# Simple-Robotics/LoIK

Measured on AMD Instinct MI355X. Metric: IK solves/sec to 1e-6 residual, Talos humanoid, batch=65536 per GPU, higher is better.
Workload: dtype f64

## Files before the change

### loik_amd/csrc/loik_device.hpp

```cpp
#pragma once

#include <hip/hip_runtime.h>

namespace loikb {

constexpr int WAVE = 64;

enum : int {
  JP_CS = 0,
  JP_V = 1,
  JP_F = 4,
  JP_G = 7,
  JP_WZ = 10,
  JP_NUS = 11,
  JP_P = 12,
  JP_R = 15,
  JP_LBUB = 16,
  JP_UD = 17,
  JREC = 20,
  JP_NPERSIST = 12,
  CP_Y = 0,
  CP_ATY = 3,
  CP_B = 6,
  CP_ATB = 9,
  CREC_SHARED_A = 12,
  CP_A = 12,
  CP_ATA = 30,
  CREC_FULL = 42,
  SP_MU = 0,
  SP_BI = 1,
  SP_ST = 2,
  SP_TAG = 3,
  SP_FLIP = 4,
  SP_SCAL = 5,
  SREC = 20,
};

struct Layout {
  int nb, nc;
  int crec;
  int off_c;
  int off_s;
  int tile_pairs;
};

enum : int {
  JF_PARENT_ROOT = 2,
  JF_MASSLESS = 4,
  JF_NOQ = 8,
  JF_REVOLUTE = 16,
  JF_CS_DIRECT = 32,
  JF_HELICAL = 64,
};

enum : int { ROT_X = 0, ROT_Y = 1, ROT_Z = 2, ROT_U = 3, ROT_NONE = 4, ROT_FREE = 5, ROT_SPH = 6, ROT_TRANS = 7, ROT_PLANAR = 8 };

struct JointDesc {
  double Rp[9];
  double tp[3];
  double axis[3];
  int parent;
  int flags;
  int cslot;
  int rot;
  double pitch;
};

enum : int { ST_CONVERGED = 1, ST_PRIMAL_INF = 2, ST_TAIL = 4, ST_DONE = 8,
             ST_PFULL = 16 };

enum : int {
  MODE_FIXED_ITERS = 1,
  MODE_CACHE_H = 2,
  MODE_A_SHARED = 4,
  MODE_BND_SHARED = 8,
  MODE_MU_OSQP = 16,
  MODE_ZERO_STATE = 32,
  MODE_FLAT_PREP = 64,
};


enum : int {
  SC_PRIMAL_RES = 0, SC_DUAL_RES, SC_PRIMAL_RES_TASK, SC_PRIMAL_RES_SLACK, SC_DUAL_RES_V, SC_DUAL_RES_NU,
  SC_TOL_PRIMAL, SC_TOL_DUAL, SC_MU, SC_MU_EQ, SC_MU_INEQ,
  SC_DELTA_X_QP, SC_DELTA_Z_QP, SC_DELTA_Y_QP, SC_AT_DELTA_Y_QP, SC_UB_DY_PLUS, SC_LB_DY_MINUS,
  SC_DELTA_FIS, SC_DELTA_YIS, SC_DELTA_W, SC_DELTA_VIS, SC_DELTA_NU,
  SC_AV_INF, SC_NU_INF, SC_HREF_V_INF, SC_G_INF, SC_STF_PLUS_W_INF,
  SC_COND1, SC_COND2, SC_TAIL_ITER,
  NSCAL
};
static_assert(SP_SCAL + (NSCAL + 1) / 2 <= SREC, "scalar record too small");

template <typename T>
struct Params {
  T Href[36];
  T Hv[6];
  T Hv_inf_norm;
  const T* href_tab;
  T rho, mu0, mu_scale;
  T tol_abs, tol_rel, tol_primal_inf, tol_tail_solve;
  int max_iter;
  int mode;
  int B;
  int max_launch_iters;
  Layout L;
};

template <typename T>
struct Bufs {
  char* tiles;
  const T* uni;
  unsigned int* counters;
  int* wave_live;
  double* log;
  int* log_rows;
  int log_cap, log_B;
};

template <typename T> struct Vec2;
template <> struct Vec2<double> { using type = double2; };
template <> struct Vec2<float> { using type = float2; };

template <typename T>
__host__ __device__ constexpr size_t pair_bytes() { return (size_t)WAVE * 2 * sizeof(T); }

template <typename T>
__device__ __forceinline__ typename Vec2<T>::type ldp(const char* rec, int p)
{
  return *reinterpret_cast<const typename Vec2<T>::type*>(rec + (size_t)p * pair_bytes<T>());
}
template <typename T>
__device__ __forceinline__ void stp(char* rec, int p, T x, T y)
{
  typename Vec2<T>::type v;
  v.x = x; v.y = y;
  *reinterpret_cast<typename Vec2<T>::type*>(rec + (size_t)p * pair_bytes<T>()) = v;
}
template <typename T>
__device__ __forceinline__ void st_lo(char* rec, int p, T x) { *reinterpret_cast<T*>(rec + (size_t)p * pair_bytes<T>()) = x; }
template <typename T>
__device__ __forceinline__ void st_hi(char* rec, int p, T x) { *reinterpret_cast<T*>(rec + (size_t)p * pair_bytes<T>() + sizeof(T)) = x; }

template <typename T>
__device__ __forceinline__ void ld6(const char* rec, int p, T* x)
{
#pragma unroll
  for (int k = 0; k < 3; ++k) {
    const typename Vec2<T>::type v = ldp<T>(rec, p + k);
    x[2 * k] = v.x; x[2 * k + 1] = v.y;
  }
}
template <typename T>
__device__ __forceinline__ void st6(char* rec, int p, const T* x)
{
#pragma unroll
  for (int k = 0; k < 3; ++k) stp<T>(rec, p + k, x[2 * k], x[2 * k + 1]);
}

__host__ __device__ constexpr int sym(int i, int j)
{
  return (i <= j) ? (i * 6 - (i * (i - 1)) / 2 + (j - i)) : (j * 6 - (j * (j - 1)) / 2 + (i - j));
}

__host__ __device__ __forceinline__ double tabs(double x) { return __builtin_fabs(x); }
__host__ __device__ __forceinline__ float tabs(float x) { return __builtin_fabsf(x); }
__host__ __device__ __forceinline__ double tmax(double a, double b) { return __builtin_fmax(a, b); }
__host__ __device__ __forceinline__ float tmax(float a, float b) { return __builtin_fmaxf(a, b); }
__host__ __device__ __forceinline__ double tmin(double a, double b) { return __builtin_fmin(a, b); }
__host__ __device__ __forceinline__ float tmin(float a, float b) { return __builtin_fminf(a, b); }

template <typename T>
__device__ __forceinline__ bool update_mu(int mode, T primal, T dual, T norm_p, T norm_d, T& mu, int& kexp)
{
  if (mode & MODE_MU_OSQP) {
    const T rp = primal / (norm_p + T(1e-10)), rd = dual / (norm_d + T(1e-10));
    T mu_new = mu * (T)__builtin_sqrt((double)(rp / (rd + T(1e-10))));
    mu_new = tmin(tmax(mu_new, T(1e-6)), T(1e6));
    if (mu_new > T(5.0) * mu || mu_new < T(0.2) * mu) { mu = mu_new; return true; }
    return false;
  }
  if (primal > T(10) * dual) { mu *= T(10); ++kexp; return true; }
  if (dual > T(10) * primal) { mu *= T(0.1); --kexp; return true; }
  return false;
}

template <typename T>
__device__ __forceinline__ T inf6(const T* x)
{
  T m = tabs(x[0]);
#pragma unroll
  for (int k = 1; k < 6; ++k) m = tmax(m, tabs(x[k]));
  return m;
}

template <typename T>
__device__ __forceinline__ void cross3(const T* a, const T* b, T* o)
{
  o[0] = a[1] * b[2] - a[2] * b[1];
  o[1] = a[2] * b[0] - a[0] * b[2];
  o[2] = a[0] * b[1] - a[1] * b[0];
}

template <typename T>
__device__ __forceinline__ void mat3_vec(const T* A, const T* x, T* y)
{
#pragma unroll
  for (int i = 0; i < 3; ++i) y[i] = A[3 * i] * x[0] + A[3 * i + 1] * x[1] + A[3 * i + 2] * x[2];
}

template <typename T>
__device__ __forceinline__ void mat3t_vec(const T* A, const T* x, T* y)
{
#pragma unroll
  for (int i = 0; i < 3; ++i) y[i] = A[i] * x[0] + A[3 + i] * x[1] + A[6 + i] * x[2];
}

template <typename T>
__device__ __forceinline__ void make_liMi(const JointDesc& d, T c, T s, T* R, T* t)
{
  T Rp[9], tp[3], ax[3];
#pragma unroll
  for (int k = 0; k < 9; ++k) Rp[k] = (T)d.Rp[k];
#pragma unroll
  for (int k = 0; k < 3; ++k) { tp[k] = (T)d.tp[k]; ax[k] = (T)d.axis[k]; }
  if (d.flags & JF_REVOLUTE) {
    if (d.rot == ROT_X) {
#pragma unroll
      for (int i = 0; i < 3; ++i) {
        R[3 * i] = Rp[3 * i];
        R[3 * i + 1] = Rp[3 * i + 1] * c + Rp[3 * i + 2] * s;
        R[3 * i + 2] = Rp[3 * i + 2] * c - Rp[3 * i + 1] * s;
// ... 1518 lines not shown
```

### loik_amd/csrc/loik_flat_prep.hpp

```cpp
#pragma once

#include "loik_lean.hpp"

namespace loikb {

enum : int { C2_LANE = 0, C2_B = 2, C2_Y = 8, C2_ATYW = 14 , C2_ATBW = 20,
             C2_ATYF = 26 , C2_CW = 32, C2_DLT = 38 ,
             C2_VC = 44 , C2_ATY = 50 , C2_AW = 56, C2_AWT = 92,
             C2_A = 128, C2D = 164 };

constexpr int PREP_G = 32;
enum : int { PR_RT = 0, PR_JS = PR_RT + 12 * PREP_G, PR_SW = PR_JS + 4 * PREP_G, PR_SC = PR_SW + 3 * WAVE, PR_C = PR_SC + 32 };
enum : int { PRS_BNORM = 0, PRS_TGIN = 1, PRS_STY = 2, PRS_MU = 11, PRS_KEXP, PRS_ITER, PRS_STATUS, PRS_TAILIT, PRS_FLIP, PRS_N };

__host__ __device__ __forceinline__ int flat_prep_stride(int nc) { return PR_C + nc * C2D; }

template <typename T>
__device__ __forceinline__ T prep_awy_of(const T* blk, int k)
{
  const T* r = blk + C2_AW + 6 * k;
  const T* y = blk + C2_Y;
  return ((r[0] * y[0] + r[1] * y[1]) + r[2] * y[2]) + ((r[3] * y[3] + r[4] * y[4]) + r[5] * y[5]);
}
template <typename T>
__device__ __forceinline__ T prep_aty_of(const T* blk, int k)
{
  const T* A_ = blk + C2_A + k;
  const T* y = blk + C2_Y;
  return ((A_[0] * y[0] + A_[6] * y[1]) + A_[12] * y[2]) + ((A_[18] * y[3] + A_[24] * y[4]) + A_[30] * y[5]);
}

constexpr int PREP_NC = 4;
static_assert((WAVE / PREP_G) * PREP_NC * C2D <= (WAVE + 1) * 22, "the constraint blocks are built in k_fslots' placement rows");

template <typename T>
struct FlatPrepIn {
  typename Vec2<T>::type nus, lu;
  T sc;
  T cv[PREP_NC];
  T ca[PREP_NC][2];
};
template <typename T>
__device__ __forceinline__ void flat_prep_fetch(FlatPrepIn<T>& in, bool has_inst, const Params<T>& P, const Bufs<T>& Bf, const char* ip, const char* rec,
                                                int jlane, bool isj_lane)
{
  const Layout& L = P.L;
  in.nus.x = in.nus.y = T(0); in.lu.x = in.lu.y = T(0);
  in.sc = T(0);
#pragma unroll
  for (int c = 0; c < PREP_NC; ++c) { in.cv[c] = T(0); in.ca[c][0] = in.ca[c][1] = T(0); }
  if (!has_inst) return;
  if (isj_lane) {
    in.nus = ldp<T>(rec, JP_NUS);
    if (!(P.mode & MODE_BND_SHARED)) in.lu = ldp<T>(rec, JP_LBUB);
  }
  if (jlane < PRS_N) {
    const char* srec = ip + (size_t)L.off_s * pair_bytes<T>();
    const int sc_i = jlane == 3 ? SC_TOL_PRIMAL : jlane == 4 ? SC_TOL_DUAL : jlane == 5 ? SC_DELTA_Y_QP : jlane == 6 ? SC_AT_DELTA_Y_QP
                   : jlane == 7 ? SC_UB_DY_PLUS : jlane == 8 ? SC_LB_DY_MINUS : jlane == 9 ? SC_COND1 : jlane == 10 ? SC_COND2
                   : jlane == PRS_TAILIT ? SC_TAIL_ITER : -1;
    const int pair = sc_i >= 0 ? SP_SCAL + sc_i / 2
                   : jlane == PRS_BNORM || jlane == PRS_ITER ? SP_BI : jlane == PRS_TGIN ? SP_TAG : jlane == PRS_STY || jlane == PRS_STATUS ? SP_ST
                   : jlane == PRS_FLIP ? SP_FLIP : SP_MU;
    const int hi = sc_i >= 0 ? (sc_i & 1) : (jlane == PRS_ITER || jlane == PRS_STY || jlane == PRS_KEXP) ? 1 : 0;
    in.sc = *reinterpret_cast<const T*>(srec + (size_t)pair * pair_bytes<T>() + (size_t)hi * sizeof(T));
  }
#pragma unroll
  for (int c = 0; c < PREP_NC; ++c) {
    if (c >= L.nc) break;
    const char* crec = ip + (size_t)(L.off_c + c * L.crec) * pair_bytes<T>();
    if (jlane < 18) {
      const int which = jlane / 6, k = jlane % 6;
      const int pair = which == 0 ? CP_B : which == 1 ? CP_Y : CP_ATY;
      in.cv[c] = *reinterpret_cast<const T*>(crec + (size_t)(pair + k / 2) * pair_bytes<T>() + (k & 1) * sizeof(T));
    }
#pragma unroll
    for (int i = 0; i < 2; ++i) {
      const int e = jlane + i * PREP_G;
      if (e < LCA)
        in.ca[c][i] = (P.mode & MODE_A_SHARED) ? Bf.uni[c * LCA + e]
                                               : *reinterpret_cast<const T*>(crec + (size_t)(CP_A + e / 2) * pair_bytes<T>() + (e & 1) * sizeof(T));
    }
  }
}

template <typename T>
__device__ __forceinline__ void flat_prep_write(T* __restrict__ blk, bool has_inst, const Params<T>& P, const FlatPrepIn<T>& in, int jlane, int cslot,
                                                const T* R0, const T* t0, const T* Sw, T* cb)
{
  const Layout& L = P.L;
  if (has_inst) {
#pragma unroll
    for (int k = 0; k < 9; ++k) blk[PR_RT + k * PREP_G + jlane] = R0[k];
#pragma unroll
    for (int k = 0; k < 3; ++k) blk[PR_RT + (9 + k) * PREP_G + jlane] = t0[k];
#pragma unroll
    for (int k = 0; k < 3; ++k) { blk[PR_SW + k * WAVE + jlane] = Sw[k]; blk[PR_SW + k * WAVE + PREP_G + jlane] = Sw[3 + k]; }
    blk[PR_JS + jlane] = in.nus.x; blk[PR_JS + PREP_G + jlane] = in.nus.y;
    blk[PR_JS + 2 * PREP_G + jlane] = in.lu.x; blk[PR_JS + 3 * PREP_G + jlane] = in.lu.y;
    if (jlane < PRS_N) blk[PR_SC + jlane] = in.sc;
  }
  const int nce = L.nc * C2D;
  for (int e = jlane; e < nce; e += PREP_G) cb[e] = T(0);
  tail_sync();
#pragma unroll
  for (int c = 0; c < PREP_NC; ++c) {
    if (c >= L.nc || !has_inst) break;
    T* c_ = cb + c * C2D;
    if (jlane < 18) {
      const int which = jlane / 6, k = jlane % 6;
      c_[(which == 0 ? C2_B : which == 1 ? C2_Y : C2_ATY) + k] = in.cv[c];
    }
    c_[C2_A + jlane] = in.ca[c][0];
    if (jlane + PREP_G < LCA) c_[C2_A + PREP_G + jlane] = in.ca[c][1];
  }
  if (cslot >= 0) cb[cslot * C2D + C2_LANE] = (T)jlane;
  tail_sync();
  if (cslot >= 0) {
    T* c_ = cb + cslot * C2D;
    const T* A_ = c_ + C2_A;
#pragma unroll
    for (int q = 0; q < 6; ++q) {
      T aj[6], o[6];
#pragma unroll
      for (int k = 0; k < 6; ++k) aj[k] = A_[6 * q + k];
      act_force(R0, t0, aj, o);
#pragma unroll
      for (int k = 0; k < 6; ++k) { c_[C2_AW + 6 * k + q] = o[k]; c_[C2_AWT + 6 * q + k] = o[k]; }
    }
    T ay[6], o[6];
#pragma unroll
    for (int k = 0; k < 6; ++k) ay[k] = c_[C2_ATY + k];
    act_force(R0, t0, ay, o);
#pragma unroll
    for (int k = 0; k < 6; ++k) c_[C2_ATYW + k] = o[k];
  }
  tail_sync();
  if (jlane < 6 * L.nc) {
    const int ccl = jlane / 6, k = jlane - 6 * ccl;
    T* const ccb = cb + ccl * C2D;
    T ab = T(0);
#pragma unroll
    for (int q = 0; q < 6; ++q) ab += ccb[C2_AW + 6 * k + q] * ccb[C2_B + q];
    ccb[C2_ATBW + k] = ab;
    const T aw = prep_awy_of<T>(ccb, k), at = prep_aty_of<T>(ccb, k);
    ccb[C2_CW + k] = ccb[C2_ATYW + k] - aw;
    ccb[C2_DLT + k] = at - ccb[C2_ATY + k];
  }
  tail_sync();
  if (has_inst)
    for (int e = jlane; e < nce; e += PREP_G) blk[PR_C + e] = cb[e];
}

}
```

### loik_amd/csrc/loik_host.hip

```cpp
#include "loik_device.hpp"
#include "loik_tail.hpp"
#include "loik_lean.hpp"
#include "loik_flat.hpp"
#include "loik_flat2.hpp"
#include "loik_passes.hpp"
#include "loik_pose.hpp"
#include "loik_pose_tasks.hpp"
#include "loik_pose_multistart.hpp"
#include "loik_pose_path.hpp"
#include "loik_pose_track.hpp"
#include "loik_pose_accel.hpp"
#include "loik_pose_step.hpp"
#include "loik_pose_jacobian.hpp"
#include "loik_pose_collision.hpp"
#include "loik_pose_grid.hpp"
#include "loik_pose_motion.hpp"
#include "loik_pose_shortcut.hpp"
#include "loik_pose_retime.hpp"
#include "loik_pose_blend.hpp"
#include "loik_pose_plan.hpp"
#include "loik_pose_avoid.hpp"
#include "loik_flat_inst.hpp"
#include "loik_devmem.hpp"
#ifdef LOIKB_FLAT_SEPARATE_TU
LOIKB_FLAT2_INSTANCES(LOIKB_FLAT2_DECL)
LOIKB_FLAT1_INSTANCES(LOIKB_FLAT1_DECL)
#ifdef LOIKB_TAIL_PROF
int loikb_flat_prof_read(unsigned long long* out, int which, int reset);
#endif
#endif

#include "../../include/loik_amd.h"
#include "../../include/loik_amd_pose.h"
#include "../../include/loik_amd_limits.h"
#include "../../include/loik_amd_tasks.h"
#include "../../include/loik_amd_multistart.h"
#include "../../include/loik_amd_path.h"
#include "../../include/loik_amd_track.h"
#include "../../include/loik_amd_accel.h"
#include "../../include/loik_amd_step.h"
#include "../../include/loik_amd_axis.h"
#include "../../include/loik_amd_jacobian.h"
#include "../../include/loik_amd_collision.h"
#include "../../include/loik_amd_motion.h"
#include "../../include/loik_amd_avoid.h"
#include "../../include/loik_amd_shortcut.h"
#include "../../include/loik_amd_retime.h"
#include "../../include/loik_amd_blend.h"
#include "../../include/loik_amd_plan.h"
#include "../../include/loik_amd_grid.h"

#include <algorithm>
#include <atomic>
#include <chrono>
#include <cmath>
#include <cstdio>
#include <cstdlib>
#include <cstring>
#include <limits>
#include <mutex>
#include <string>
#include <thread>
#include <vector>

using namespace loikb;

static thread_local std::string g_last_error;

#define HIPCHK(expr)                                                                                       \
  do {                                                                                                     \
    hipError_t _e = (expr);                                                                                \
    if (_e != hipSuccess) {                                                                                \
      char _buf[512];                                                                                      \
      snprintf(_buf, sizeof(_buf), "%s failed: %s (%s:%d)", #expr, hipGetErrorString(_e), __FILE__, __LINE__); \
      g_last_error = _buf;                                                                                 \
      return LOIKB_ERR_HIP;                                                                                \
    }                                                                                                      \
  } while (0)

#define BUFCHK(expr)                                                                                       \
  do {                                                                                                     \
    if (!(expr)) {                                                                                         \
      char _buf[512];                                                                                      \
      snprintf(_buf, sizeof(_buf), "%s failed: %s (%s:%d)", #expr, hipGetErrorString(hipGetLastError()), __FILE__, __LINE__); \
      g_last_error = _buf;                                                                                 \
      return LOIKB_ERR_HIP;                                                                                \
    }                                                                                                      \
  } while (0)

namespace {

std::atomic<unsigned long long> g_devmem[4];
inline bool count_alloc(bool ok, int k, size_t bytes) { if (ok) { ++g_devmem[k]; g_devmem[k + 1] += bytes; } return ok; }
inline void count_free(int k, size_t bytes) { --g_devmem[k]; g_devmem[k + 1] -= bytes; }
struct DeviceMem {
  static bool allocate(void** out, size_t bytes) { return count_alloc(hipMalloc(out, bytes) == hipSuccess, 0, bytes); }
  static void free(void* p, size_t bytes) { (void)hipFree(p); count_free(0, bytes); }
};
struct PinnedMem {
  static bool allocate(void** out, size_t bytes) { return count_alloc(hipHostMalloc(out, bytes) == hipSuccess, 2, bytes); }
  static void free(void* p, size_t bytes) { (void)hipHostFree(p); count_free(2, bytes); }
};
template <class T = void> using DevBuf = OwnedBuf<DeviceMem, T>;
template <class T = void> using PinBuf = OwnedBuf<PinnedMem, T>;

constexpr int ROWMAP_CAP = 8192;

struct Tuning {
  int team = MAX_TEAM;
  int team_max = 1 << 30;
  int tile_pad = -1;
  bool lean = true;
  bool flat = true;
  bool flat_split = true;
  int flat_win_lo = 0, flat_win_n = 0;
  int flat_build = 2;
  int flat_small_batch = 2048;
  int flat_min_batch = 1;
  int small_finish = 1;
  int flat_slice = -1;
  bool flat_prep = true;
  bool flat_zero_state = true;
  int flat_order_holdoff = 4;
  bool flat_order = true;
  int tail_waves = TAIL_WAVES;
  int lean_decades = 10;
  int lean_klo = -2;
  int lean_wg_per_cu = 0;
  int lean_wg_waves = 0;
  bool lean_adapt = true;
  double compact_ratio = 0.85;
  bool direct_tail = true;
  int lat_iters = 16;
  int chunks = 0;
  bool trace = false;
  void read_env()
  {
    auto geti = [](const char* n, int& v) { if (const char* e = getenv(n)) v = atoi(e); };
    geti("LOIKB_TEAM", team); team = std::max(1, std::min(MAX_TEAM, team));
    geti("LOIKB_TEAM_MAX", team_max);
    geti("LOIKB_TILE_PAD", tile_pad);
    if (const char* e = getenv("LOIKB_LEAN")) lean = atoi(e) != 0;
    if (const char* e = getenv("LOIKB_FLAT")) flat = atoi(e) != 0;
    if (!lean) flat = false;
    if (const char* e = getenv("LOIKB_FLAT_SPLIT")) flat_split = atoi(e) != 0;
    if (const char* e = getenv("LOIKB_FLAT_BUILD")) flat_build = std::max(0, std::min(2, atoi(e)));
    if (const char* e = getenv("LOIKB_FLAT_WINDOW")) { if (sscanf(e, "%d,%d", &flat_win_lo, &flat_win_n) != 2) flat_win_n = 0; }
    if (const char* e = getenv("LOIKB_FLAT_SLICE")) flat_slice = std::min(65535, std::max(-1, atoi(e)));
    if (const char* e = getenv("LOIKB_FLAT_MIN_BATCH")) flat_min_batch = std::max(1, atoi(e));
    if (const char* e = getenv("LOIKB_SMALL_FINISH")) small_finish = atoi(e);
    if (const char* e = getenv("LOIKB_FLAT_SMALL_BATCH")) flat_small_batch = std::max(0, atoi(e));
    if (const char* e = getenv("LOIKB_FLAT_ORDER")) flat_order = atoi(e) != 0;
    if (const char* e = getenv("LOIKB_FLAT_ZERO_STATE")) flat_zero_state = atoi(e) != 0;
    if (const char* e = getenv("LOIKB_FLAT_PREP")) flat_prep = atoi(e) != 0;
    if (const char* e = getenv("LOIKB_FLAT_ORDER_HOLDOFF")) flat_order_holdoff = std::max(0, atoi(e));
    geti("LOIKB_TAIL_WAVES", tail_waves); tail_waves = std::max(1, std::min(TAIL_WAVES, tail_waves));
    geti("LOIKB_LEAN_DECADES", lean_decades); lean_decades = std::max(1, std::min(15, lean_decades));
    geti("LOIKB_LEAN_KLO", lean_klo);
    geti("LOIKB_LEAN_WG_PER_CU", lean_wg_per_cu);
    geti("LOIKB_LEAN_WG_WAVES", lean_wg_waves);
    if (const char* e = getenv("LOIKB_LEAN_ADAPT")) lean_adapt = atoi(e) != 0;
    if (const char* e = getenv("LOIKB_COMPACT_RATIO")) compact_ratio = atof(e);
    direct_tail = getenv("LOIKB_NO_DIRECT_TAIL") == nullptr;
    geti("LOIKB_LAT_ITERS", lat_iters);
    geti("LOIKB_CHUNKS", chunks);
    trace = getenv("LOIKB_TRACE") != nullptr;
  }
};

struct EnginePlan {
  bool flat = false;
  const char* why_not_flat = "";
  int flat_waves_cu = 0;
  bool lean = false;
  const char* why_not_lean = "";
  int lean_waves_cu = 0, lean_wg_waves = TAIL_WAVES;
  int ndec = 10, kexp_lo = -2;
  int tail_max = 32768;
  int nchunks = 1;
  bool solve_ok = true;
  size_t solve_lds_need = 0;
};

struct loikb_solver_impl {
  Tuning tune;
  EnginePlan plan;
  int nj = 0, nb = 0, nq = 0, nv = 0;
  std::vector<int> parents, jtype, idx_q, idx_v;
  std::vector<JointDesc> jd;
  int ext_nj = 0;
  std::vector<int> link_of, first_of;
  std::vector<int> lim_q, dof_ext, dof_jt;
  int* d_link_sel = nullptr;
  int* d_first_sel = nullptr;
  struct TeamSched {
    int nw = 1, T_up = 0, T_down = 0, nslots = 0, nvslots = 0;
    std::vector<StepDesc> up, down;
    std::vector<int> rlist;
    StepDesc *d_up = nullptr, *d_down = nullptr;
    int* d_rlist = nullptr;
  } sched[2];
  std::vector<TailTopo> topo;
  std::vector<int> child_list;
  int maxdepth = 0, maxchild = 0;
  int multi_from = 1;
  TailTopo* d_topo = nullptr;
  int* d_child_list = nullptr;
  struct FlatSched {
    bool ok = false;
    const char* why = "";
    int G = 0, nanc = 0, nscan = 0, njmp = 0;
    int fblk = 0;
    std::vector<FlatLane> lanes;
    FlatLane* d_lanes = nullptr;
  } flat;
  bool ud_stale = false;
  loikb_options opt{};
  int B = 0, nc = 0;
  size_t esz = 8;
  bool f32 = false;
  double Href[36]{}, vref[6]{}, Hv[6]{};
  double Hv_inf_norm = 0.0;
  std::vector<double> href_tab;
  double mu_start = 0.0;
  bool per_link = false;
  void* d_href = nullptr;
  double* d_href64 = nullptr;
  std::vector<float> href_tab32;
  std::vector<int> active_ids;
  int nc_active = 0;
  std::vector<double> A_host;
  bool have_problem = false;
  bool have_q = false;
  bool a_shared = true, bnd_shared = true;
  bool href_diag = true;
  int device = 0;
  int ncu = 256;
  hipStream_t stream = nullptr;
  hipStream_t own_stream = nullptr;
  hipEvent_t ev_t0 = nullptr, ev_t1 = nullptr;
  std::vector<DevBuf<>> allocs;
  std::mutex alloc_mu;
  JointDesc* d_jd = nullptr;
  int* d_idx_q = nullptr;
  int* d_rowmap = nullptr;
  int* d_rowmap_scratch = nullptr;
  struct RowmapEntry { std::vector<int> rm; int* d; };
  std::vector<RowmapEntry> rowmap_cache;
  bool defer_sync = false;
  bool offer_queue = false;
  PinBuf<char> h_pin;
  size_t pin_cap = 0, pin_off = 0;
  std::vector<double> uni_host;
  bool uni_dirty = false;
  std::vector<int> cslots_on_device;
  double* d_q = nullptr;
  void* d_uni = nullptr;
  DevBuf<> d_stage;
  DevBuf<> d_getscr[2];
  struct ResMap { DevBuf<int> d; int key[6] = {-1, -1, -1, -1, -1, -1}; int n = 0; int off[8] = {0, 0, 0, 0, 0, 0, 0, 0}; };
  ResMap resmaps[4];
  int resmap_next = 0;
  PinBuf<double> h_res;
  Layout L{};
  struct Set {
    char* tiles = nullptr;
    int ntiles = 0;
    DevBuf<char> tiles_mem;
    DevBuf<int> map, wave_live, wave_off;
  };
  Set home;
  struct Chunk {
    int first_tile = 0, B = 0;
    Set set[3];
    hipStream_t stream = nullptr;
    bool own_stream = false;
    hipEvent_t ev_k0 = nullptr, ev_k1 = nullptr, ev_k2 = nullptr;
    DevBuf<unsigned int> d_counters;
    PinBuf<unsigned int> h_counters;
    DevBuf<int> d_slots;
    DevBuf<int> d_slots2;
    DevBuf<int> d_order;
    DevBuf<unsigned int> d_order_bins;
    int order_n = 0;
    unsigned long long order_epoch = 0;
    int order_holdoff = 0;
    int arrival_n = 0;
    double arrival_ms = 0.0;
    DevBuf<int> d_ring;
    int ring_cap = 0;
    DevBuf<> d_hslots;
    DevBuf<> d_fslots;
    DevBuf<> d_park;
    DevBuf<> d_prep;
    DevBuf<unsigned int> d_fmask;
    DevBuf<void*> d_aux;
    const void* aux_h[4] = {nullptr, nullptr, nullptr, nullptr};
    std::vector<int> h_wave;
    loikb_stats stats{};
    bool unfinished_counted = false;
    bool queue_ready = false;
    bool small_finished = false;
    int rc = 0;
    std::string err;
    std::vector<std::pair<float, float>> solve_iv, tail_iv;
  };
  std::vector<Chunk> chunks;
  hipEvent_t ev_fork = nullptr;
  loikb_stats stats{};
  bool pass_active = false;
  bool zero_state = false;
  unsigned long long inputs_epoch = 1;
  bool href_known = false;
  bool tab_bcast = false;
  double tab_H[36] = {0}, tab_v[6] = {0};
  int log_truncated = 0;
  PassLayout PL{};
  DevBuf<double> d_pass;
  DevBuf<int> d_pass_cslot;
  int seen_lo = 1 << 20, seen_hi = -(1 << 20);
  unsigned long long end_hist[32] = {0}, end_hist_n = 0;
  unsigned long long solve_serial = 0, end_hist_epoch = 0;
  DevBuf<double> d_log;
  DevBuf<int> d_log_rows;
  int log_rows_cap = 0;
  bool have_log = false;
  struct PoseState {
    double* d_tgt = nullptr;
    double* d_b = nullptr;
    double* d_err = nullptr;
    double* d_A = nullptr;
    int* d_status = nullptr;
    int* d_steps = nullptr;
    int* d_clink = nullptr;
    unsigned int* d_count = nullptr;
    int nc = 0;
    double timing[4] = {0, 0, 0, 0};
    bool have_limits = false;
    bool flags_valid = false;
    std::vector<PoseLimit> lim;
    PoseLimit* d_lim = nullptr;
    int* d_lflags = nullptr;
    unsigned char* d_inrange = nullptr;
    double2* d_box = nullptr;
    bool have_accel = false;
    bool vel_valid = false;
    bool have_v0 = false;
    std::vector<double> a_max;
    double* d_amax = nullptr;
    double* d_zp = nullptr;
    double* d_v0 = nullptr;
    double* d_vout = nullptr;
    const int* vel_status = nullptr;
    bool have_step = false;
    bool step_valid = false;
    loikb_step_params step = {0.5, 1e-4, 6, 0, 0};
    double* d_trial = nullptr;
    double* d_alpha = nullptr;
    int* d_backtracks = nullptr;
    int* d_failed = nullptr;
    int* d_frun = nullptr;
    bool have_tasks = false;
    std::vector<PoseTask> tasks;
    PoseTask* d_tasks = nullptr;
    bool have_dex = false;
    loikb_dexterity_params dex = {1.0, 0};
    struct Collision {
      std::vector<int> links;
      std::vector<int> car, scar;
      int ns = 0, nws = 0, nwb = 0;
      bool self_on = false;
      std::vector<int> ignore;
      std::vector<unsigned short> pairs;
      DevBuf<double> d_sph, d_wsph, d_wbox;
      DevBuf<int> d_scar, d_car;
      DevBuf<unsigned short> d_pairs;
      DevBuf<double> d_place;
      DevBuf<double> d_mslab;
      bool have_grid = false;
      int gn[3] = {0, 0, 0};
      double go[3] = {0.0, 0.0, 0.0}, gh = 0.0;
      DevBuf<unsigned int> d_grid, d_grid_next;
      DevBuf<unsigned char> d_occ;
      bool have_ms = false;
      loikb_clearance_params ms = {0.0, 0};
    } col;
    struct Avoid {
      bool have = false;
      loikb_avoid_params prm = {0.0, 0.0, 1.0, 0};
      bool valid = false;
      DevBuf<double> d_minseen;
      DevBuf<int> d_asteps, d_aflags;
      DevBuf<double> d_place;
      DevBuf<double> d_base;
    } avoid;
  } pose;
  struct MultiStartState {
    bool have_ranges = false;
    std::vector<double> lo, hi, w;
    std::vector<double> up_lo, up_hi;
    std::vector<int> up_table;
    double* d_tgt_in = nullptr;
    double* d_tgt = nullptr;
    double* d_q0 = nullptr;
    int* d_table = nullptr;
    int* d_dofq = nullptr;
    double *d_lo = nullptr, *d_hi = nullptr, *d_w = nullptr;
    int* d_round = nullptr;
    int *d_winner = nullptr, *d_gstatus = nullptr, *d_nreached = nullptr;
    double *d_cost = nullptr, *d_wq = nullptr, *d_werr = nullptr;
    unsigned int* d_count = nullptr;
    double* d_dex = nullptr;
    double* d_dexcost = nullptr;
    double* d_dexfr = nullptr;
    int* d_dexrows = nullptr;
    std::vector<double> dex_fr;
    std::vector<int> dex_rows;
    double* d_clr = nullptr;
    int* d_clrwit = nullptr;
    int* d_lstatus = nullptr;
    double *d_iclr = nullptr, *d_wclr = nullptr;
    int *d_wwit = nullptr, *d_nclear = nullptr;
    bool clr_valid = false;
    int G = 0, nc = 0;
    double timing[6] = {0, 0, 0, 0, 0, 0};
  } ms;
  struct PathState {
    int* d_cursor = nullptr;
    int* d_ws = nullptr;
    int* d_wfrom = nullptr;
    int* d_lstatus = nullptr;
    int* d_pstatus = nullptr;
    DevBuf<double> d_wp;
    DevBuf<int> d_wsteps;
    DevBuf<double> d_Q;
    int T = 0;
    bool recorded = false;
    double timing[4] = {0, 0, 0, 0};
  } path;
  struct TrackState {
    int* d_ontrack = nullptr;
    double* d_worst = nullptr;
    int* d_worst_at = nullptr;
    DevBuf<double> d_smp;
    DevBuf<double> d_errmax;
    DevBuf<int> d_inner;
    DevBuf<double> d_Q;
    DevBuf<double> d_Z;
    int T = 0;
    int record = 0;
    double timing[4] = {0, 0, 0, 0};
  } track;
};
using Chunk = loikb_solver_impl::Chunk;

template <class T>
int alloc_zeroed(loikb_solver_impl* S, DevBuf<T>& b, size_t bytes, hipStream_t st = nullptr, bool use_st = false)
{
  BUFCHK(b.regrow(bytes ? bytes : 16));
  HIPCHK(hipMemsetAsync(b, 0, b.bytes(), use_st ? st : S->stream));
  return LOIKB_OK;
}

int alloc_dev(loikb_solver_impl* S, void** out, size_t bytes, hipStream_t st = nullptr, bool use_st = false)
// ... 417 lines not shown
    const int i = l + 1;
    F.depth = depth[i]; F.size = size[i];
    int a = i;
    for (int dist = 0, r = 0; a > 0; a = parents[a], ++dist) {
      if (dist > 0) F.anc[depth[a] - 1] = a - 1;
      if (dist == (1 << r) && r < FLAT_JMP) F.jmp[r++] = a - 1;
    }
  }
  std::vector<int> free_lanes;
  for (int l = G - 1; l >= 0; --l)
    if (l >= nb || size[l + 1] == 1) free_lanes.push_back(l);
  for (int l = 0; l < nb; ++l) {
    const int m = size[l + 1] - 1, k = depth[l + 1] - 1;
    int nparts = 0;
    for (int c0 = 0; c0 < m; c0 += FLAT_RED) {
      int owner = l;
      if (c0 > 0) {
        if (free_lanes.empty() || nparts >= FLAT_PART) { out.why = "a joint with too many descendants for the flat engine's reduction schedule"; out.lanes.clear(); return; }
        owner = free_lanes.back(); free_lanes.pop_back();
        out.lanes[owner].helper = 1;
        out.lanes[l].part[nparts++] = owner;
      }
      for (int t = 0; t < FLAT_RED && c0 + t < m; ++t) out.lanes[owner].red[t] = k * G + (l + 1 + c0 + t);
    }
  }
  out.G = G; out.nanc = std::max(1, maxdepth - 1); out.nscan = nscan; out.njmp = njmp;
  int col = 0;
  for (int l = 0; l < G; ++l) {
    out.lanes[l].helper |= col << 8;
    col += out.lanes[l].depth;
  }
  out.fblk = (std::max(FSLOT_ROWS * G, col) + 1) & ~1;
  out.ok = true;
}

template <typename T>
Bufs<T> make_bufs(loikb_solver_impl* S, Chunk* C, int k)
{
  Bufs<T> Bf{};
  Bf.tiles = C->set[k].tiles;
  Bf.uni = (const T*)S->d_uni;
  Bf.counters = C->d_counters;
  Bf.wave_live = C->set[k].wave_live;
  Bf.log = S->d_log; Bf.log_rows = S->d_log_rows; Bf.log_cap = S->log_rows_cap; Bf.log_B = S->B;
  return Bf;
}

static void jacobi6(double* a, double* ev)
{
  for (int sweep = 0; sweep < 50; ++sweep) {
    double off = 0.0;
    for (int p = 0; p < 6; ++p)
      for (int q = p + 1; q < 6; ++q) off += a[6 * p + q] * a[6 * p + q];
    if (off < 1e-300) break;
    for (int p = 0; p < 6; ++p)
      for (int q = p + 1; q < 6; ++q) {
        const double apq = a[6 * p + q];
        if (apq == 0.0) continue;
        const double theta = (a[6 * q + q] - a[6 * p + p]) / (2.0 * apq);
        const double t = (theta >= 0.0 ? 1.0 : -1.0) / (std::fabs(theta) + std::sqrt(theta * theta + 1.0));
        const double c = 1.0 / std::sqrt(t * t + 1.0), sn = t * c;
        for (int k = 0; k < 6; ++k) {
          const double akp = a[6 * k + p], akq = a[6 * k + q];
          a[6 * k + p] = c * akp - sn * akq;
          a[6 * k + q] = sn * akp + c * akq;
        }
        for (int k = 0; k < 6; ++k) {
          const double apk = a[6 * p + k], aqk = a[6 * q + k];
          a[6 * p + k] = c * apk - sn * aqk;
          a[6 * q + k] = sn * apk + c * aqk;
        }
      }
  }
  for (int k = 0; k < 6; ++k) ev[k] = a[7 * k];
}

static double spectral_mu0(const loikb_solver_impl* S)
{
  double lo = 0.0, hi = 0.0;
  bool any = false;
  for (int i = 1; i < S->nj; ++i) {
    if (S->jd[i].flags & JF_MASSLESS) continue;
    const double* H = S->href_tab.data() + (size_t)i * HREF_ROW;
    double m[36], ev[6];
    for (int r = 0; r < 6; ++r)
      for (int c = 0; c < 6; ++c) m[6 * r + c] = 0.5 * (H[6 * r + c] + H[6 * c + r]) + (r == c ? S->opt.rho : 0.0);
    jacobi6(m, ev);
    for (int k = 0; k < 6; ++k) {
      if (!any || ev[k] < lo) lo = ev[k];
      if (!any || ev[k] > hi) hi = ev[k];
      any = true;
    }
  }
  if (!any) return S->opt.mu;
  lo = std::max(lo, S->opt.rho);
  hi = std::max(hi, lo);
  if (!(lo > 0.0)) return S->opt.mu;
  const long q = std::lround(4.0 * std::log10(std::sqrt(lo * hi)));
  return std::min(1e6, std::max(1e-6, std::pow(10.0, (double)q / 4.0)));
}

static double solve_mu0(const loikb_solver_impl* S)
{
  return S->opt.mu_update_strat == LOIKB_MU_MAXEIGENVALUE && S->mu_start > 0.0 ? S->mu_start : S->opt.mu;
}

template <typename T>
Params<T> make_params(loikb_solver_impl* S)
{
  Params<T> P{};
  for (int k = 0; k < 36; ++k) P.Href[k] = (T)S->Href[k];
  for (int k = 0; k < 6; ++k) P.Hv[k] = (T)S->Hv[k];
  P.Hv_inf_norm = (T)S->Hv_inf_norm;
  P.href_tab = S->per_link ? (const T*)S->d_href : nullptr;
  P.rho = (T)S->opt.rho; P.mu0 = (T)solve_mu0(S); P.mu_scale = (T)S->opt.mu_equality_scale_factor;
  P.tol_abs = (T)S->opt.tol_abs; P.tol_rel = (T)S->opt.tol_rel; P.tol_primal_inf = (T)S->opt.tol_primal_inf;
  P.tol_tail_solve = (T)S->opt.tol_tail_solve;
  P.max_iter = S->opt.max_iter;
  int mode = 0;
  if (S->opt.flags & LOIKB_OPT_FIXED_ITERS) mode |= MODE_FIXED_ITERS;
  if (!(S->opt.flags & LOIKB_OPT_NO_H_CACHE)) mode |= MODE_CACHE_H;
  if (S->a_shared) mode |= MODE_A_SHARED;
  if (S->bnd_shared) mode |= MODE_BND_SHARED;
  if (S->opt.mu_update_strat == LOIKB_MU_OSQP) mode |= MODE_MU_OSQP;
  P.mode = mode;
  P.B = S->B;
  P.max_launch_iters = S->opt.max_iter + 1;
  P.L = S->L;
  return P;
}

int reset_home(loikb_solver_impl* S, int what, bool with_queue = false)
{
  const dim3 grid(S->home.ntiles), block(WAVE);
  if (what & RS_SOLVER) S->zero_state = (what & (RS_DATA_COLD | RS_RECURSION)) != 0;
  if (with_queue && !S->f32 && S->chunks.size() == 1 && S->tune.small_finish && S->tune.flat_split && S->B <= S->tune.flat_small_batch &&
      S->chunks[0].d_ring != nullptr && S->chunks[0].d_slots != nullptr && S->chunks[0].d_counters != nullptr) {
    loikb_solver_impl::Chunk& C = S->chunks[0];
    const int qblocks = (std::max(C.ring_cap, NCOUNTERS) + WAVE - 1) / WAVE;
    hipLaunchKernelGGL(k_reset_and_queue<double>, dim3(S->home.ntiles + qblocks), block, 0, S->stream, S->home.tiles, S->L, what, (double)solve_mu0(S),
                       S->home.ntiles, C.d_ring, C.ring_cap, C.d_slots, S->B, C.d_counters, NCOUNTERS);
    HIPCHK(hipGetLastError());
    C.queue_ready = true;
    return LOIKB_OK;
  }
  with_real(S, [&](auto t) {
    using T = decltype(t);
    hipLaunchKernelGGL(k_reset<T>, grid, block, 0, S->stream, S->home.tiles, S->L, what, (T)solve_mu0(S));
  });
  HIPCHK(hipGetLastError());
  return LOIKB_OK;
}

int to_device(loikb_solver_impl* S, const void* src, size_t bytes, bool src_device, const void** out)
{
  if (src_device) { *out = src; return LOIKB_OK; }
  if (S->defer_sync && bytes <= ((size_t)64 << 10)) {
    if (!S->h_pin) {
      if (S->h_pin.regrow((size_t)512 << 10)) S->pin_cap = S->h_pin.bytes();
      else (void)hipGetLastError();
    }
    const size_t need = (bytes + 255) & ~(size_t)255;
    if (S->h_pin && S->pin_off + need <= S->pin_cap) {
      memcpy(S->h_pin + S->pin_off, src, bytes);
      *out = S->h_pin + S->pin_off;
      S->pin_off += need;
      return LOIKB_OK;
    }
  }
  BUFCHK(S->d_stage.regrow(bytes));
  HIPCHK(hipMemcpyAsync(S->d_stage, src, bytes, hipMemcpyHostToDevice, S->stream));
  *out = S->d_stage;
  return LOIKB_OK;
}

int set_rowmap(loikb_solver_impl* S, const std::vector<int>& rm)
{
  if ((int)rm.size() > ROWMAP_CAP) { g_last_error = "row map too large"; return LOIKB_ERR_ARG; }
  for (const loikb_solver_impl::RowmapEntry& e : S->rowmap_cache)
    if (e.rm == rm) { S->d_rowmap = e.d; return LOIKB_OK; }
  if (S->d_rowmap_scratch == nullptr) S->d_rowmap_scratch = S->d_rowmap;
  if (S->rowmap_cache.size() < 64 && !rm.empty()) {
    void* p = nullptr;
    int rc = alloc_dev(S, &p, sizeof(int) * rm.size());
    if (rc) return rc;
    HIPCHK(hipMemcpyAsync(p, rm.data(), sizeof(int) * rm.size(), hipMemcpyHostToDevice, S->stream));
    HIPCHK(hipStreamSynchronize(S->stream));
    S->rowmap_cache.push_back(loikb_solver_impl::RowmapEntry{rm, (int*)p});
    S->d_rowmap = (int*)p;
    return LOIKB_OK;
  }
  S->d_rowmap = S->d_rowmap_scratch;
  HIPCHK(hipMemcpyAsync(S->d_rowmap, rm.data(), sizeof(int) * rm.size(), hipMemcpyHostToDevice, S->stream));
  HIPCHK(hipStreamSynchronize(S->stream));
  return LOIKB_OK;
}

int upload_rows(loikb_solver_impl* S, const double* src, const std::vector<int>& rm, bool src_device, bool shared)
{
  const int n = (int)rm.size();
  const void* dsrc = nullptr;
  int rc;
  if ((rc = set_rowmap(S, rm))) return rc;
  if ((rc = to_device(S, src, sizeof(double) * (shared ? (size_t)n : (size_t)S->B * n), src_device && !shared, &dsrc))) return rc;
  with_real(S, [&](auto t) {
    hipLaunchKernelGGL(k_upload_rows<decltype(t)>, grid1(S->B), dim3(256), 0, S->stream, (const double*)dsrc, n, (int)shared,
                       S->d_rowmap, S->L, S->B, S->home.tiles);
  });
  HIPCHK(hipGetLastError());
  if (!S->defer_sync) HIPCHK(hipStreamSynchronize(S->stream));
  return LOIKB_OK;
}

int upload_uni(loikb_solver_impl* S, int offset, const double* src, int n)
{
  if (S->f32) {
    std::vector<float> tmp(n);
    for (int k = 0; k < n; ++k) tmp[k] = (float)src[k];
    HIPCHK(hipMemcpyAsync((float*)S->d_uni + offset, tmp.data(), sizeof(float) * n, hipMemcpyHostToDevice, S->stream));
    HIPCHK(hipStreamSynchronize(S->stream));
  } else {
    const size_t total = (size_t)(S->nc > 0 ? S->nc : 1) * 57 + 2 * (size_t)S->nb;
    if (S->uni_host.size() != total) S->uni_host.assign(total, 0.0);
    memcpy(S->uni_host.data() + offset, src, sizeof(double) * n);
    if (S->defer_sync) { S->uni_dirty = true; return LOIKB_OK; }
    HIPCHK(hipMemcpyAsync((double*)S->d_uni + offset, src, sizeof(double) * n, hipMemcpyHostToDevice, S->stream));
    HIPCHK(hipStreamSynchronize(S->stream));
  }
  return LOIKB_OK;
}

int flush_uni(loikb_solver_impl* S)
{
  if (!S->uni_dirty) return LOIKB_OK;
  S->uni_dirty = false;
  HIPCHK(hipMemcpyAsync(S->d_uni, S->uni_host.data(), sizeof(double) * S->uni_host.size(), hipMemcpyHostToDevice, S->stream));
  return LOIKB_OK;
}

int upload_jd(loikb_solver_impl* S)
{
  HIPCHK(hipMemcpyAsync(S->d_jd, S->jd.data(), sizeof(JointDesc) * S->nj, hipMemcpyHostToDevice, S->stream));
  for (auto& sc : S->sched) {
    for (StepDesc& sd : sc.up) if (sd.joint) sd.d = S->jd[sd.joint];
    for (StepDesc& sd : sc.down) if (sd.joint) sd.d = S->jd[sd.joint];
    HIPCHK(hipMemcpyAsync(sc.d_up, sc.up.data(), sizeof(StepDesc) * sc.up.size(), hipMemcpyHostToDevice, S->stream));
    HIPCHK(hipMemcpyAsync(sc.d_down, sc.down.data(), sizeof(StepDesc) * sc.down.size(), hipMemcpyHostToDevice, S->stream));
  }
  HIPCHK(hipStreamSynchronize(S->stream));
  return LOIKB_OK;
}

int fwd_pass_init(loikb_solver_impl* S, const double* q, int in_flags)
{
  ++S->inputs_epoch;
  if (q) {
    const bool shared = in_flags & LOIKB_Q_SHARED;
    const bool dev = (in_flags & LOIKB_IN_DEVICE) && !shared;
    const void* dq = nullptr;
    int rc = to_device(S, q, sizeof(double) * (shared ? (size_t)S->nq : (size_t)S->B * S->nq), dev, &dq);
    if (rc) return rc;
    const long long elems = (long long)S->B * std::max(S->nq, S->nb);
    if (elems <= (1 << 16)) {
      const dim3 g((unsigned)((elems + 255) / 256));
      with_real(S, [&](auto t) {
        hipLaunchKernelGGL(k_set_q_fk_small<decltype(t)>, g, dim3(256), 0, S->stream, S->d_q, (const double*)dq, (int)shared, S->nq, S->d_jd,
                           S->d_idx_q, S->L, S->B, S->home.tiles);
      });
      HIPCHK(hipGetLastError());
      if (!dev && !S->defer_sync) HIPCHK(hipStreamSynchronize(S->stream));
      S->have_q = true;
      return reset_home(S, RS_HCACHE | (S->opt.warm_start ? 0 : RS_Y), S->offer_queue);
    }
    with_real(S, [&](auto t) {
      hipLaunchKernelGGL(k_advance_q<decltype(t)>, grid1(S->B), dim3(256), 0, S->stream, S->d_q, (const double*)dq, (int)shared,
                         S->nq, S->d_jd, S->d_idx_q, S->L, S->B, S->home.tiles, 0.0);
    });
    HIPCHK(hipGetLastError());
    if (!dev && !S->defer_sync) HIPCHK(hipStreamSynchronize(S->stream));
    S->have_q = true;
  } else if (!S->have_q) {
    g_last_error = "no configurations resident on the device yet (call SolveInit / Solve with a q first)";
    return LOIKB_ERR_STATE;
  }
  with_real(S, [&](auto t) {
    hipLaunchKernelGGL(k_fk_init<decltype(t)>, grid1(S->B), dim3(256), 0, S->stream, (const double*)S->d_q, S->nq, 0,
                       S->d_jd, S->d_idx_q, S->L, S->B, S->home.tiles);
  });
  HIPCHK(hipGetLastError());
  return reset_home(S, RS_HCACHE | (S->opt.warm_start ? 0 : RS_Y), S->offer_queue);
}

int constraint_products(loikb_solver_impl* S, int c_lo, int c_hi, bool grow_only)
{
  if (int frc = flush_uni(S)) return frc;
  with_real(S, [&](auto t) {
    using T = decltype(t);
    hipLaunchKernelGGL(k_constraint_products<T>, grid1(S->B), dim3(256), 0, S->stream, S->home.tiles, S->L,
                       (const T*)S->d_uni, (int)S->a_shared, c_lo, c_hi, S->B, (int)grow_only);
  });
  HIPCHK(hipGetLastError());
  return LOIKB_OK;
}

int upload_shared_A(loikb_solver_impl* S, const double* A, int c)
{
// ... 453 lines not shown
{
  const int b = blockIdx.x * blockDim.x + threadIdx.x;
  int hit = 0;
  if (b < B) {
    char* sp = lane_ptr<T>(tiles, L, b);
    const int status = (int)ldp<T>(sp + (size_t)L.off_s * pair_bytes<T>(), SP_ST).x;
    hit = !(status & (ST_CONVERGED | ST_PRIMAL_INF));
  }
  const unsigned long long m = __ballot(hit);
  if ((threadIdx.x & (WAVE - 1)) == 0 && m) atomicAdd(counter, (unsigned int)__popcll(m));
}

template <typename T>
__global__ void k_sum_iters(char* tiles, Layout L, int B, unsigned long long* __restrict__ sum)
{
  const int b = blockIdx.x * blockDim.x + threadIdx.x;
  unsigned long long it = 0;
  if (b < B) {
    char* sp = lane_ptr<T>(tiles, L, b);
    it = (unsigned long long)ldp<T>(sp + (size_t)L.off_s * pair_bytes<T>(), SP_BI).y;
  }
  for (int off = WAVE / 2; off > 0; off >>= 1) it += __shfl_down(it, off);
  if ((threadIdx.x & (WAVE - 1)) == 0 && it) atomicAdd(sum, it);
}

template <typename T>
int compact(loikb_solver_impl* S, Chunk* C, int src, int dst, int n_src, int* n_dst_out)
{
  loikb_solver_impl::Set& A = C->set[src];
  const int nw = (n_src + WAVE - 1) / WAVE;
  int rc;
  if (dst >= 0 && (rc = alloc_set(S, C->set[dst], C->set[0].ntiles, C->stream, true))) return rc;
  C->h_wave.resize(2 * (size_t)nw + 2);
  int* cnt = C->h_wave.data();
  int* off = cnt + nw + 1;
  int total = 0;
  if (dst >= 0) {
    HIPCHK(hipMemcpyAsync(cnt, A.wave_live, sizeof(int) * nw, hipMemcpyDeviceToHost, C->stream));
    HIPCHK(hipStreamSynchronize(C->stream));
    for (int w = 0; w < nw; ++w) { off[w] = total; total += cnt[w]; }
    HIPCHK(hipMemcpyAsync(A.wave_off, off, sizeof(int) * nw, hipMemcpyHostToDevice, C->stream));
  }
  MovePlan M{};
  M.src = A.tiles;
  M.dst_live = dst >= 0 ? C->set[dst].tiles : nullptr;
  M.dst_home = src == 0 ? nullptr : C->set[0].tiles;
  M.L = S->L;
  M.n_src = n_src;
  M.move_bounds = !S->bnd_shared;
  M.map_src = src == 0 ? nullptr : A.map;
  M.map_dst = dst >= 0 ? C->set[dst].map : nullptr;
  M.wave_off = A.wave_off;
  M.force_home = dst < 0;
  hipLaunchKernelGGL(k_move<T>, dim3(nw), dim3(WAVE), 0, C->stream, M);
  HIPCHK(hipGetLastError());
  HIPCHK(hipStreamSynchronize(C->stream));
  if (n_dst_out) *n_dst_out = total;
  return LOIKB_OK;
}

int lean_waves_per_cu(const loikb_solver_impl* S)
{
  const int G = lanes_per_instance(S);
  const size_t per_wave = S->f32 ? lean_lds_bytes<float>(S->nc, G, S->a_shared) : lean_lds_bytes<double>(S->nc, G, S->a_shared);
  return (int)std::min<size_t>(8, (160 * 1024) / per_wave);
}

static bool order_usable(const loikb_solver_impl* S, const Chunk* C, int n_cur)
{
  if (!S->tune.flat_order || C->order_n != n_cur) return false;
  if (C->order_epoch == S->inputs_epoch) return true;
  return (S->opt.flags & LOIKB_OPT_ORDER_FROM_PREVIOUS) && C->order_holdoff == 0;
}

void plan_engines(loikb_solver_impl* S)
{
  EnginePlan pl;
  pl.ndec = S->tune.lean_decades;
  pl.kexp_lo = S->tune.lean_klo;
  if (S->opt.flags & LOIKB_OPT_FIXED_ITERS) { pl.ndec = 1; pl.kexp_lo = 0; }
  pl.lean_waves_cu = S->nb <= WAVE ? lean_waves_per_cu(S) : 0;
  pl.lean_wg_waves = 1;
  if (S->tune.lean_wg_waves > 0 && pl.lean_waves_cu % S->tune.lean_wg_waves == 0) pl.lean_wg_waves = S->tune.lean_wg_waves;
  const char* never = S->opt.logging ? "logging = 1: every solve runs on the pass-by-pass implementation"
                      : S->opt.tail_max_instances < 0 ? "tail_max_instances < 0: the caller asked for the solve kernel alone"
                      : (S->opt.flags & LOIKB_OPT_NO_COMPACTION) ? "LOIKB_OPT_NO_COMPACTION: the solve kernel keeps every instance in its tile" : nullptr;
  if (never) pl.why_not_lean = never;
  else if (!S->tune.lean) pl.why_not_lean = "LOIKB_LEAN=0";
  else if (S->nb > WAVE) pl.why_not_lean = "more joints than lanes of a wavefront";
  else if (S->maxchild > 4) pl.why_not_lean = "a joint with more than four children";
  else if (S->opt.flags & LOIKB_OPT_NO_H_CACHE) pl.why_not_lean = "LOIKB_OPT_NO_H_CACHE (no precomputed H)";
  else if (S->opt.mu_update_strat == LOIKB_MU_OSQP) pl.why_not_lean = "OSQP penalty rule: mu is off the decade grid";
  else if (S->nb <= 16 && !(S->f32 && (S->opt.flags & LOIKB_OPT_F32_ACCURATE)) && S->B <= 32768)
    pl.why_not_lean = "a small robot (<= 16 joints): k_solve + k_tail are faster on its short solves";
  else if (pl.lean_waves_cu < 7) pl.why_not_lean = "constraint blocks leave too few wavefronts per CU in LDS";
  else pl.lean = true;
  if (S->flat.ok) {
    const size_t per_wave = S->flat.nanc <= FLAT_NA_SMALL ? flat_lds_bytes<double, FLAT_NA_SMALL>(S->nc, S->flat.G, S->a_shared, false)
                                                           : flat_lds_bytes<double, FLAT_MAXA>(S->nc, S->flat.G, S->a_shared, false);
    pl.flat_waves_cu = (int)std::min<size_t>(8, (160 * 1024) / per_wave);
    if (flat_takes_diagonal(S)) {
      const size_t pw = flat_kind(S) == FlatKind::Flat2 ? flat2_lds_bytes<FLAT_NA_SMALL>(S->nc, true)
                        : S->flat.nanc <= FLAT_NA_SMALL ? flat1_lds_bytes<FLAT_NA_SMALL>(S->nc, true, 1)
                                                        : flat1_lds_bytes<FLAT_MAXA>(S->nc, true, 1);
      pl.flat_waves_cu = std::max(pl.flat_waves_cu, (int)std::min<size_t>(8, (160 * 1024) / pw));
    }
  }
  const char* never_flat = S->opt.tail_max_instances < 0 ? never : (S->opt.flags & LOIKB_OPT_NO_COMPACTION) ? never : nullptr;
  if (never_flat) pl.why_not_flat = never_flat;
  else if (!S->tune.flat) pl.why_not_flat = S->tune.lean ? "LOIKB_FLAT=0" : "LOIKB_LEAN=0";
  else if (!S->flat.ok) pl.why_not_flat = S->flat.why;
  else if (S->f32) pl.why_not_flat = "fp32 solver";
  else if (S->opt.flags & LOIKB_OPT_NO_H_CACHE) pl.why_not_flat = "LOIKB_OPT_NO_H_CACHE (no precomputed factors)";
  else if (flat_any_mu(S) && !flat_any_mu_ok(S))
    pl.why_not_flat = "OSQP penalty rule: mu is off the decade grid, and the in-wave builder is k_flat2's / k_flat1's (17..64 joints, fp64, no logging)";
  else if (S->nb <= 16) pl.why_not_flat = "a small robot (<= 16 joints): k_solve + k_tail are faster on its short solves";
  else if (S->nc > (flat_takes_diagonal(S) ? 10 : S->flat.G / 6)) pl.why_not_flat = "more task constraints than the flat engine's lanes update in one pass";
  else if (pl.flat_waves_cu < (flat_takes_diagonal(S) ? 4 : 6)) pl.why_not_flat = "constraint blocks leave too few wavefronts per CU in LDS";
  else pl.flat = true;
  const bool flat_usable = pl.flat && (!S->href_known || flat_takes_diagonal(S) || href_is_scalar(S));
  pl.tail_max = S->opt.tail_max_instances > 0 ? S->opt.tail_max_instances : ((pl.lean || flat_usable) ? (1 << 20) : 32768);
  const int ntiles = (S->B + WAVE - 1) / WAVE;
  pl.nchunks = (ntiles >= 512 && !pl.lean && !flat_usable) ? 2 : 1;
  if (S->tune.chunks > 0) pl.nchunks = S->tune.chunks;
  pl.nchunks = std::max(1, std::min(pl.nchunks, ntiles));
  {
    auto need_of = [&](const loikb_solver_impl::TeamSched& sc) {
      const int edge = std::max(std::max(sc.nslots, 1) * EDGE_ENT, sc.nw > 1 ? sc.nw * Norms<double>::NALL : 0);
      return (size_t)(edge + std::max(sc.nvslots, 1) * 6) * WAVE * S->esz;
    };
    pl.solve_lds_need = need_of(S->sched[0]);
    pl.solve_ok = pl.solve_lds_need <= (size_t)160 * 1024;
    if (!pl.solve_ok) { pl.tail_max = 1 << 20; pl.nchunks = 1; }
  }
  S->plan = pl;
}

static int batch_tail_max(const loikb_solver_impl* S)
{
  return S->opt.tail_max_instances > 0 ? S->opt.tail_max_instances : S->plan.tail_max;
}

static bool direct_tail_of(const loikb_solver_impl* S, int n, int tail_max)
{
  return S->nb <= WAVE && S->opt.tail_max_instances >= 0 && S->opt.max_launch_iters <= 0 &&
         !(S->opt.flags & (LOIKB_OPT_NO_COMPACTION | LOIKB_OPT_NO_H_CACHE)) && n <= tail_max && S->tune.direct_tail;
}

static bool bushy_goes_on_chip(const loikb_solver_impl* S)
{
  return direct_tail_of(S, S->B, std::max(1, batch_tail_max(S)));
}

template <typename T>
struct TailCtx {
  loikb_solver_impl* S; Chunk* C; Params<T>& P; Bufs<T> Bf;
  loikb_solver_impl::Set& A; int cur, n_cur;
  bool whole_set, small_flat;
  int G, ipw;
  int ndec, kexp_lo;
  const int* list; int n;
  double total_ms = 0.0;
  unsigned long long iters = 0;
};

struct OrderUse { bool ordered = false, was_stale = false; };

static int take_up_order(const loikb_solver_impl* S, Chunk* C, bool eligible, bool count_down, int n_cur, OrderUse* use)
{
  use->ordered = eligible && order_usable(S, C, n_cur);
  use->was_stale = use->ordered && C->order_epoch != S->inputs_epoch;
  if (count_down && C->order_holdoff > 0) --C->order_holdoff;
  if (use->ordered) HIPCHK(hipMemcpyAsync(C->d_slots, C->d_order, sizeof(int) * (size_t)n_cur, hipMemcpyDeviceToDevice, C->stream));
  C->stats.flat_ordered += use->ordered ? 1 : 0;
  return LOIKB_OK;
}

template <typename T>
static int leave_order(const loikb_solver_impl* S, Chunk* C, const loikb_solver_impl::Set& A, int n_cur, bool flat_engine)
{
  HIPCHK(hipMemsetAsync(C->d_order_bins, 0, sizeof(unsigned int) * 2 * ORDER_BINS, C->stream));
  hipLaunchKernelGGL(k_order_count<T>, grid1(n_cur), dim3(256), 0, C->stream, A.tiles, S->L, n_cur, S->opt.max_iter, C->d_order_bins,
                     flat_engine ? C->d_counters + ORDER_DEC_HIST : (unsigned int*)nullptr);
  if (flat_engine) HIPCHK(hipMemcpyAsync(C->h_counters, C->d_counters, NCOUNTERS * sizeof(unsigned int), hipMemcpyDeviceToHost, C->stream));
  hipLaunchKernelGGL(k_order_scan, dim3(1), dim3(ORDER_BINS), 0, C->stream, C->d_order_bins);
  hipLaunchKernelGGL(k_order_scatter<T>, grid1(n_cur), dim3(256), 0, C->stream, A.tiles, S->L, n_cur, S->opt.max_iter, C->d_order_bins, C->d_order);
  HIPCHK(hipGetLastError());
  C->order_n = n_cur;
  C->order_epoch = S->inputs_epoch;
  return LOIKB_OK;
}

static void judge_order(const loikb_solver_impl* S, Chunk* C, int n_cur, OrderUse use, double ms)
{
  if (C->arrival_n != n_cur) { C->arrival_n = n_cur; C->arrival_ms = 0.0; }
  if (!use.ordered) C->arrival_ms = ms;
  else if (use.was_stale && C->arrival_ms > 0.0 && ms > 0.985 * C->arrival_ms) C->order_holdoff = S->tune.flat_order_holdoff;
}

static void record_decades(loikb_solver_impl* S, unsigned int seen, int kexp_lo, unsigned int escaped)
{
  for (int d = 0; d < 16; ++d)
    if (seen & (1u << d)) { S->seen_lo = std::min(S->seen_lo, kexp_lo + d); S->seen_hi = std::max(S->seen_hi, kexp_lo + d); }
  if (escaped) { S->seen_lo = S->plan.kexp_lo; S->seen_hi = S->plan.kexp_lo + S->plan.ndec - 1; }
}

struct FlatLaunch {
  FlatKind kind; int nanc, frows, has_hv; bool small_na;
  int mur;
  int ndec, kexp_lo, dw0, nw;
  int slice;
  bool prep;
  double cu_sh; dim3 grid;
};

static int flat_launch_slice(const loikb_solver_impl* S, const Chunk* C, FlatKind kind, int mur, int n, int n_cur, bool ordered)
{
  if (kind == FlatKind::Flat) return 0;
  if (kind == FlatKind::Flat1) return mur == 1 ? 0 : flat_slice_for(S, n, ordered);
  int q = flat_slice_for(S, n, ordered);
  if (q > 0 && (!C->d_park || (size_t)n_cur * flat2_park_stride(S->nc, true) * sizeof(double) > C->d_park.bytes())) q = 0;
  if (mur == 1 && S->tune.flat_slice < 0) q = 0;
  return q;
}

static void flat_table_window(const loikb_solver_impl* S, FlatLaunch& F, int n)
{
  int wlo = 0, whi = -1;
  const bool win_ok = F.slice > 0;
  if (S->tune.flat_win_n > 0) { wlo = S->tune.flat_win_lo; whi = wlo + S->tune.flat_win_n - 1; }
  else if (S->tune.flat_build == 2 && win_ok && S->end_hist_n > 0) {
    unsigned long long cum = 0;
    int k03 = 99, k97 = 99;
    for (int k = 0; k < 32; ++k) {
      cum += S->end_hist[k];
      if (k03 == 99 && cum * 100 >= 3ull * S->end_hist_n) k03 = k - 16;
      if (k97 == 99 && cum * 100 >= 97ull * S->end_hist_n) k97 = k - 16;
    }
    wlo = std::min(0, k03); whi = std::max(0, k97);
  }
  else if (S->tune.flat_build == 2 && win_ok && n >= 49152) {
    wlo = 0; whi = 4;
  }
  const int lo = std::max(wlo, F.kexp_lo), hi = std::min(whi, F.kexp_lo + F.ndec - 1);
  if (hi >= lo && (hi - lo + 1) < F.ndec) { F.dw0 = lo - F.kexp_lo; F.nw = hi - lo + 1; }
  else if (S->tune.flat_build == 2) F.mur = 0;
}

template <typename T>
static int launch_flat_kernel(TailCtx<T>& X, FlatLaunch& F)
{
  loikb_solver_impl* S = X.S; Chunk* C = X.C;
  const int n = X.n, has_hv = F.has_hv;
  const int cus = (int)(F.cu_sh + 0.5);
  if (one_per_wave(F.kind)) {
    BUFCHK(C->d_aux.regrow(4 * sizeof(void*)));
    const void* auxh[4] = {S->d_topo, S->d_child_list, C->d_fmask, C->d_prep.as<double>()};
    if (memcmp(auxh, C->aux_h, sizeof(auxh)) != 0) {
      memcpy(C->aux_h, auxh, sizeof(auxh));
      HIPCHK(hipStreamSynchronize(C->stream));
      HIPCHK(hipMemcpy(C->d_aux, C->aux_h, sizeof(auxh), hipMemcpyHostToDevice));
    }
  }
  const Params<double>& Pd = *reinterpret_cast<const Params<double>*>(&X.P);
  const Bufs<double>& Bd = *reinterpret_cast<const Bufs<double>*>(&X.Bf);
  const FlatVariant v = flat_variant(F.kind, href_mode(S), F.slice > 0, S->opt.logging != 0, F.mur);
  const int quantum = v.sliced ? F.slice : 0;
  if (F.kind == FlatKind::Flat2) {
    const size_t lds2 = flat2_lds_bytes<FLAT_NA_SMALL>(S->nc, has_hv != 0, F.mur == 1);
    int per_cu = (int)std::min<size_t>((size_t)8, (160 * 1024) / lds2);
    if (S->tune.lean_wg_per_cu > 0) per_cu = std::min(per_cu, S->tune.lean_wg_per_cu);
    F.grid = dim3((unsigned)std::min(n, per_cu * cus));
    const int win_bits = (int)(((F.nw >= 16 ? 0xFFFFu : ((1u << F.nw) - 1u)) << F.dw0) & 0xFFFFu);
    hipLaunchKernelGGL(flat_kernel(FLAT2_TABLE, v, FLAT_NA_SMALL), F.grid, dim3(WAVE), lds2, C->stream, Pd, Bd, (const JointDesc*)S->d_jd, (const FlatLane*)S->flat.d_lanes,
                       F.nanc, S->flat.nscan, S->flat.njmp, C->d_ring, n, C->d_fslots.as<const double>(), F.frows, F.kexp_lo, F.ndec, (double)S->Href[0],
                       (int)((unsigned int)has_hv | ((unsigned int)(S->maxdepth & 0xFF) << 8) | ((unsigned int)win_bits << 16)), C->ring_cap - 1,
                       quantum, C->d_park.as<double>(), flat2_park_stride(S->nc, true), (const void* const*)C->d_aux);
  } else if (F.kind == FlatKind::Flat1) {
    auto lds_of = [&](int bufs) { return F.small_na ? flat1_lds_bytes<FLAT_NA_SMALL>(S->nc, has_hv != 0, bufs) : flat1_lds_bytes<FLAT_MAXA>(S->nc, has_hv != 0, bufs); };
    const int one_buf = F.mur != 1 && std::min<size_t>(8, (160 * 1024) / lds_of(1)) > std::min<size_t>(8, (160 * 1024) / lds_of(2));
    const size_t lds1 = lds_of(one_buf ? 1 : 2);
    int per_cu1 = (int)std::min<size_t>(8, (160 * 1024) / lds1);
    if (S->tune.lean_wg_per_cu > 0) per_cu1 = std::min(per_cu1, S->tune.lean_wg_per_cu);
    F.grid = dim3((unsigned)std::min(n, per_cu1 * cus));
    hipLaunchKernelGGL(flat_kernel(FLAT1_TABLE, v, F.small_na ? FLAT_NA_SMALL : FLAT_MAXA), F.grid, dim3(WAVE), lds1, C->stream, Pd, Bd, (const JointDesc*)S->d_jd,
                       (const FlatLane*)S->flat.d_lanes, F.nanc, S->flat.nscan, S->flat.njmp, C->d_ring, n, C->d_fslots.as<const double>(), F.frows,
                       F.kexp_lo, F.ndec, (double)S->Href[0], has_hv | (one_buf ? 2 : 0) | ((S->maxdepth & 0xFF) << 8), C->ring_cap - 1, quantum,
                       (const void* const*)C->d_aux);
  } else {
    const size_t flds = F.small_na ? flat_lds_bytes<T, FLAT_NA_SMALL>(S->nc, X.G, S->a_shared, has_hv) : flat_lds_bytes<T, FLAT_MAXA>(S->nc, X.G, S->a_shared, has_hv);
    int lgG = 3;
    while ((1 << lgG) < X.G) ++lgG;
    F.grid = dim3((unsigned)std::min((n + X.ipw - 1) / X.ipw, (int)std::min<size_t>(4, (160 * 1024) / flds) * cus));
    auto* kernel = S->opt.logging ? (F.small_na ? k_flat<T, FLAT_NA_SMALL, true> : k_flat<T, FLAT_MAXA, true>)
                                  : (F.small_na ? k_flat<T, FLAT_NA_SMALL> : k_flat<T, FLAT_MAXA>);
    hipLaunchKernelGGL(kernel, F.grid, dim3(WAVE), flds, C->stream, X.P, X.Bf, (const JointDesc*)S->d_jd, (const FlatLane*)S->flat.d_lanes, F.nanc,
                       S->flat.nscan, S->flat.njmp, (const int*)C->d_ring, n, lgG, C->d_fslots.as<const T>(), F.frows, F.kexp_lo, F.ndec, (T)S->Href[0], has_hv);
  }
  HIPCHK(hipGetLastError());
  return LOIKB_OK;
}

template <typename T>
static int flat_read_back(TailCtx<T>& X, const FlatLaunch& F, OrderUse use, bool order_pass, bool small_finish, bool queue_ready, int* next)
{
  loikb_solver_impl* S = X.S; Chunk* C = X.C;
  const int n_first = X.n, n_cur = X.n_cur;
  const hipEvent_t ev_first = queue_ready ? S->ev_t0 : C->ev_k0;
  float ms = 0.f, t0 = 0.f, hms = 0.f;
  HIPCHK(hipEventElapsedTime(&ms, ev_first, C->ev_k1));
  if (!queue_ready) HIPCHK(hipEventElapsedTime(&t0, S->ev_t0, C->ev_k0));
  if (!X.small_flat) HIPCHK(hipEventElapsedTime(&hms, ev_first, C->ev_k2));
  X.iters += C->h_counters[1];
  if (C->h_counters[FLAT_COUNTERS_ERR]) {
    g_last_error = (C->h_counters[FLAT_COUNTERS_ERR] & 4u) ? "internal: the flat engine's dynamic LDS does not start at LDS address 0 (lds_abs)"
                                                           : "internal: a wavefront of the flat engine gave up waiting on its work queue";
    return LOIKB_ERR_STATE;
  }
  C->stats.lean_requeues += (int)C->h_counters[LEAN_Q_REQUEUES];
  const unsigned int escaped = C->h_counters[2];
  C->stats.flat_built += (int)C->h_counters[FLAT_COUNTERS_BUILT];
  {
    std::lock_guard<std::mutex> lock(S->alloc_mu);
    record_decades(S, C->h_counters[LEAN_DECADES_SEEN], F.kexp_lo, escaped);
    if (order_pass) {
      if (S->end_hist_epoch != S->solve_serial) { S->end_hist_epoch = S->solve_serial; S->end_hist_n = 0; for (int k = 0; k < 32; ++k) S->end_hist[k] = 0; }
      for (int k = 0; k < 32; ++k) { S->end_hist[k] += C->h_counters[ORDER_DEC_HIST + k]; S->end_hist_n += C->h_counters[ORDER_DEC_HIST + k]; }
    }
    if (F.mur == 2) {
      for (int k = 0; k < 32; ++k)
        if (C->h_counters[FLAT_COUNTERS_DEC + k]) { S->seen_lo = std::min(S->seen_lo, k - 16); S->seen_hi = std::max(S->seen_hi, k - 16); }
    }
    S->ud_stale = true;
  }
  C->stats.hslots_ms += hms;
  if (C->h_counters[FLAT_COUNTERS_DRY])
    C->stats.queue_dry_ms += (double)(unsigned int)(C->h_counters[FLAT_COUNTERS_TDRY] - C->h_counters[FLAT_COUNTERS_T0]) * 1e-5;
  if (one_per_wave(F.kind) && X.whole_set && n_first == n_cur) judge_order(S, C, n_cur, use, (double)ms - (double)hms);
  if (S->tune.trace)
    fprintf(stderr, "[loikb] flat engine: %6d instances on %u workgroups, done at %8.3f ms (slots %6.3f ms)  "
                    "inst-iters %9u  wave-iters %7u  slot loads %7u (+ %u served from LDS)  escaped %u  still iterating %u%s\n",
            n_first, F.grid.x, ms, hms, C->h_counters[1], C->h_counters[5], C->h_counters[6],
            C->h_counters[FLAT_COUNTERS_SLOT_HITS], escaped, C->h_counters[3], F.prep ? "  fresh instances from prepared records" : "");
  C->stats.lean_escaped += (int)escaped;
  C->tail_iv.emplace_back(t0, t0 + ms);
  X.total_ms = ms; X.n = (int)C->h_counters[3]; X.list = next;
  if (X.n == 0 && X.whole_set && X.cur == 0 && n_first == n_cur && S->chunks.size() == 1) { C->stats.n_unfinished = (int)C->h_counters[4]; C->unfinished_counted = true; C->small_finished = small_finish; }
  return LOIKB_OK;
}

template <typename T>
static int launch_flat(TailCtx<T>& X)
{
  loikb_solver_impl* S = X.S; Chunk* C = X.C;
  Params<T>& P = X.P;
  const int n = X.n, n_cur = X.n_cur;
  const bool small_flat = X.small_flat, whole_set = X.whole_set;
  FlatLaunch F;
  F.kind = flat_kind(S); F.nanc = S->flat.nanc; F.small_na = F.nanc <= FLAT_NA_SMALL; F.has_hv = S->Hv_inf_norm != 0.0;
  F.frows = S->flat.fblk;
  F.cu_sh = std::max(1.0, S->ncu * ((double)C->B / (double)S->B));
  F.ndec = X.ndec; F.kexp_lo = X.kexp_lo; F.dw0 = 0;
  const bool can_build2 = S->tune.flat_build && F.kind == FlatKind::Flat2 && C->d_fmask != nullptr && !S->opt.logging && !S->per_link && href_is_scalar(S);
  F.mur = flat_any_mu(S) ? 1 : (can_build2 ? 2 : 0);
  if (F.mur == 1) { F.ndec = 1; F.kexp_lo = 0; }
  if (F.mur == 2) { F.ndec = S->plan.ndec; F.kexp_lo = S->plan.kexp_lo; }
  const size_t need = (size_t)n_cur * F.ndec * F.frows * sizeof(T);
  if (need > C->d_fslots.bytes()) { g_last_error = "internal: decade-slot buffer of the flat engine smaller than the chunk"; return LOIKB_ERR_STATE; }
  P.max_launch_iters = S->opt.max_iter + 1;
  const int mode_keep = P.mode;
  if (whole_set && S->zero_state && S->tune.flat_zero_state) P.mode |= MODE_ZERO_STATE;
  const bool queue_ready = small_flat && C->queue_ready && n_cur == S->B;
  C->queue_ready = false;
  if (!queue_ready && small_flat) hipLaunchKernelGGL(k_queue_init_iota, grid1(std::max(C->ring_cap, NCOUNTERS)), dim3(256), 0, C->stream, C->d_ring, C->ring_cap, C->d_slots, n_cur, C->d_counters, NCOUNTERS);
  else if (!queue_ready) HIPCHK(hipMemsetAsync(C->d_counters, 0, NCOUNTERS * sizeof(unsigned int), C->stream));
  if (!queue_ready) HIPCHK(hipEventRecord(C->ev_k0, C->stream));
  OrderUse use;
  int rc = take_up_order(S, C, !small_flat && whole_set && X.list == C->d_slots && n == n_cur && one_per_wave(F.kind), true, n_cur, &use);
  if (rc) return rc;
  F.slice = flat_launch_slice(S, C, F.kind, F.mur, n, n_cur, use.ordered);
  F.nw = F.ndec;
  if (F.mur == 2) flat_table_window(S, F, n);
  if (F.mur == 0) { F.ndec = X.ndec; F.kexp_lo = X.kexp_lo; F.nw = F.ndec; F.dw0 = 0; }
  const bool prep = F.kind == FlatKind::Flat2 && S->tune.flat_prep && F.ndec > 0 && F.mur != 1 && !S->opt.logging && whole_set && n == n_cur &&
                    flat_prep_fits(S) && X.G == PREP_G && C->d_prep && (size_t)n_cur * flat_prep_stride(S->nc) * sizeof(double) <= C->d_prep.bytes();
  if (prep) P.mode |= MODE_FLAT_PREP;
  F.prep = prep;
  if (F.ndec > 0) {
    const dim3 hgrid((unsigned)((n + X.ipw - 1) / X.ipw));
    const size_t slds = (std::max((size_t)(WAVE + 1) * 22, (size_t)((F.small_na ? FLAT_NA_SMALL : FLAT_MAXA) + 1) * WAVE) + (size_t)(WAVE + 1) * 6 +
                         (size_t)X.ipw * S->nc * 21 + 16) * sizeof(T);
    auto* fslots = F.small_na ? k_fslots<T, FLAT_NA_SMALL> : k_fslots<T, FLAT_MAXA>;
    hipLaunchKernelGGL(fslots, hgrid, dim3(WAVE), slds, C->stream, P, X.Bf, (const JointDesc*)S->d_jd, (const TailTopo*)S->d_topo,
                       (const int*)S->d_child_list, (const FlatLane*)S->flat.d_lanes, S->maxdepth, F.nanc, F.frows, S->flat.njmp, X.list, n,
                       X.G, C->d_fslots.as<T>(), F.kexp_lo, F.ndec, F.dw0, F.nw, F.mur == 2 ? C->d_fmask : (unsigned int*)nullptr,
                       prep ? C->d_prep.as<T>() : (T*)nullptr);
    HIPCHK(hipGetLastError());
  }
  if (!small_flat) HIPCHK(hipEventRecord(C->ev_k2, C->stream));
  if (!small_flat) hipLaunchKernelGGL(k_ring_fill, grid1(C->ring_cap), dim3(256), 0, C->stream, C->d_ring, C->ring_cap, X.list, n, C->d_counters);
  if ((rc = launch_flat_kernel(X, F))) return rc;
  P.mode = mode_keep;
  int* next = (X.list == C->d_slots) ? C->d_slots2 : C->d_slots;
  const bool small_finish = small_flat && S->tune.small_finish;
  if (small_finish)
    hipLaunchKernelGGL(k_small_finish<T>, dim3(1), dim3(256), 0, C->stream, X.A.tiles, S->L, X.list, n, next, C->d_counters, NCOUNTERS, C->h_counters);
  else
    hipLaunchKernelGGL(k_list_unfinished<T>, grid1(n), dim3(256), 0, C->stream, X.A.tiles, S->L, X.list, n, next, C->d_counters + 3);
  HIPCHK(hipGetLastError());
  C->stats.launches++; C->stats.tail_launches++; C->stats.lean_launches++; C->stats.flat_launches++;
  if (F.kind == FlatKind::Flat2) C->stats.flat_split_launches++;
  HIPCHK(hipEventRecord(C->ev_k1, C->stream));
  const bool order_pass = !small_flat && S->tune.flat_order && whole_set && n == n_cur && one_per_wave(F.kind) && !(S->opt.flags & LOIKB_OPT_FIXED_ITERS);
  if (!order_pass && !small_finish) HIPCHK(hipMemcpyAsync(C->h_counters, C->d_counters, NCOUNTERS * sizeof(unsigned int), hipMemcpyDeviceToHost, C->stream));
  if (order_pass && (rc = leave_order<T>(S, C, X.A, n_cur, true))) return rc;
  HIPCHK(hipStreamSynchronize(C->stream));
  return flat_read_back(X, F, use, order_pass, small_finish, queue_ready, next);
}

template <typename T>
static int launch_lean(TailCtx<T>& X)
{
  loikb_solver_impl* S = X.S; Chunk* C = X.C;
  Params<T>& P = X.P;
  const Bufs<T>& Bf = X.Bf;
  const int n = X.n, n_cur = X.n_cur, G = X.G, ipw = X.ipw, ndec = X.ndec, kexp_lo = X.kexp_lo;
  const int* list = X.list;
  const bool whole_set = X.whole_set, per_link = S->per_link;
  const size_t need = (size_t)n_cur * ndec * HSLOT_PAIRS * G * 2 * sizeof(T);
  if (need > C->d_hslots.bytes()) { g_last_error = "internal: decade-slot buffer smaller than the chunk"; return LOIKB_ERR_STATE; }
  const int waves_cu = S->plan.lean_waves_cu;
  const int ltw = S->plan.lean_wg_waves;
  const size_t lds = ltw * lean_lds_bytes<T>(S->nc, G, S->a_shared);
  if (lds > 64 * 1024) {
    HIPCHK(hipFuncSetAttribute((const void*)k_lean<T, true>, hipFuncAttributeMaxDynamicSharedMemorySize, (int)lds));
    HIPCHK(hipFuncSetAttribute((const void*)k_lean<T, false>, hipFuncAttributeMaxDynamicSharedMemorySize, (int)lds));
    HIPCHK(hipFuncSetAttribute((const void*)k_lean<T, false, true>, hipFuncAttributeMaxDynamicSharedMemorySize, (int)lds));
  }
  const int wg_per_cu = S->tune.lean_wg_per_cu > 0 ? S->tune.lean_wg_per_cu : waves_cu / ltw;
  const int wg_cap = wg_per_cu * std::max(1, (int)(S->ncu * ((double)C->B / (double)S->B) + 0.5));
  HIPCHK(hipEventRecord(C->ev_k0, C->stream));
  OrderUse use;
  int rc = take_up_order(S, C, whole_set && list == C->d_slots && n == n_cur, whole_set, n_cur, &use);
  if (rc) return rc;
  P.max_launch_iters = S->opt.max_iter + 1;
  const int wg_needed = (n + ipw * ltw - 1) / (ipw * ltw);
  const dim3 grid((unsigned)std::min(wg_needed, wg_cap));
  HIPCHK(hipMemsetAsync(C->d_counters, 0, NCOUNTERS * sizeof(unsigned int), C->stream));
  const dim3 hgrid((unsigned)((n + ipw - 1) / ipw));
  const size_t hlds = (size_t)(WAVE + 1) * 22 * sizeof(T);
  auto* hslots = per_link ? k_hslots<T, false, true> : S->href_diag ? k_hslots<T, true> : k_hslots<T, false>;
  hipLaunchKernelGGL(hslots, hgrid, dim3(WAVE), hlds, C->stream, P, Bf, (const JointDesc*)S->d_jd, (const TailTopo*)S->d_topo,
                     (const int*)S->d_child_list, S->maxdepth, S->maxchild, list, n, G, C->d_hslots.as<T>(), kexp_lo, ndec);
  HIPCHK(hipEventRecord(C->ev_k2, C->stream));
  hipLaunchKernelGGL(k_ring_fill, grid1(C->ring_cap), dim3(256), 0, C->stream, C->d_ring, C->ring_cap, list, n, C->d_counters);
  auto* lean = per_link ? k_lean<T, false, true> : S->href_diag ? k_lean<T, true> : k_lean<T, false>;
  hipLaunchKernelGGL(lean, grid, dim3(WAVE * ltw), lds, C->stream, P, Bf, (const JointDesc*)S->d_jd, (const TailTopo*)S->d_topo,
                     (const int*)S->d_child_list, S->maxdepth, S->maxchild, C->d_ring, n, G, C->d_hslots.as<const T>(), kexp_lo, ndec, S->multi_from);
  HIPCHK(hipGetLastError());
  int* next = (list == C->d_slots) ? C->d_slots2 : C->d_slots;
  hipLaunchKernelGGL(k_list_unfinished<T>, grid1(n), dim3(256), 0, C->stream, X.A.tiles, S->L, list, n, next, C->d_counters + 3);
  HIPCHK(hipGetLastError());
  HIPCHK(hipEventRecord(C->ev_k1, C->stream));
  HIPCHK(hipMemcpyAsync(C->h_counters, C->d_counters, NCOUNTERS * sizeof(unsigned int), hipMemcpyDeviceToHost, C->stream));
  const bool lean_orders = S->tune.flat_order && whole_set && n == n_cur && !(S->opt.flags & LOIKB_OPT_FIXED_ITERS);
  if (lean_orders && (rc = leave_order<T>(S, C, X.A, n_cur, false))) return rc;
  HIPCHK(hipStreamSynchronize(C->stream));
  float ms = 0.f, t0 = 0.f, hms = 0.f;
  HIPCHK(hipEventElapsedTime(&ms, C->ev_k0, C->ev_k1));
  if (lean_orders) judge_order(S, C, n_cur, use, (double)ms);
  HIPCHK(hipEventElapsedTime(&t0, S->ev_t0, C->ev_k0));
  X.iters += C->h_counters[1];
  const unsigned int escaped = C->h_counters[2];
  {
    std::lock_guard<std::mutex> lock(S->alloc_mu);
    record_decades(S, C->h_counters[LEAN_DECADES_SEEN], kexp_lo, escaped);
  }
  C->stats.lean_requeues += (int)C->h_counters[LEAN_Q_REQUEUES];
  HIPCHK(hipEventElapsedTime(&hms, C->ev_k0, C->ev_k2));
  C->stats.hslots_ms += hms;
  if (S->tune.trace)
    fprintf(stderr, "[loikb] lean engine: %6d instances on %u workgroups, done at %8.3f ms"
                    "  inst-iters %9u  wave-iters %7u slot loads %7u  escaped %u  still iterating %u  requeued %u\n",
            n, grid.x, ms, C->h_counters[1], C->h_counters[5], C->h_counters[6], escaped,
            C->h_counters[3], C->h_counters[LEAN_Q_REQUEUES]);
  C->stats.launches++; C->stats.tail_launches++; C->stats.lean_launches++;
  X.total_ms = ms; X.n = (int)C->h_counters[3]; X.list = next;
  C->tail_iv.emplace_back(t0, t0 + ms);
  C->stats.lean_escaped += (int)escaped;
  return LOIKB_OK;
}

template <typename T>
static int launch_tail_kernel(TailCtx<T>& X, int tw, size_t lds)
{
  loikb_solver_impl* S = X.S; Chunk* C = X.C;
  const int n = X.n, n_cur = X.n_cur;
  const int cu_share = std::max(1, (int)(S->ncu * (TAIL_WAVES / tw) * ((double)C->B / (double)S->B) + 0.5));
  X.P.max_launch_iters = S->opt.max_iter + 1;
  const int wg_needed = (n + X.ipw * tw - 1) / (X.ipw * tw);
  const dim3 grid((unsigned)std::min(wg_needed, cu_share));
  HIPCHK(hipMemsetAsync(C->d_counters, 0, NCOUNTERS * sizeof(unsigned int), C->stream));
  HIPCHK(hipEventRecord(C->ev_k0, C->stream));
  const bool tail_whole = X.whole_set && X.list == C->d_slots && n == n_cur && !(S->opt.flags & LOIKB_OPT_FIXED_ITERS) && S->tune.flat_order;
  OrderUse use;
  int rc = take_up_order(S, C, tail_whole, tail_whole, n_cur, &use);
  if (rc) return rc;
  auto* kernel = S->href_diag ? k_tail<T, true> : k_tail<T, false>;
  hipLaunchKernelGGL(kernel, grid, dim3(WAVE * tw), lds, C->stream, X.P, X.Bf, (const JointDesc*)S->d_jd, (const TailTopo*)S->d_topo,
                     (const int*)S->d_child_list, S->maxdepth, S->maxchild, X.list, n, X.G);
  HIPCHK(hipGetLastError());
  HIPCHK(hipEventRecord(C->ev_k1, C->stream));
  HIPCHK(hipMemcpyAsync(C->h_counters, C->d_counters, NCOUNTERS * sizeof(unsigned int), hipMemcpyDeviceToHost, C->stream));
  if (tail_whole && (rc = leave_order<T>(S, C, X.A, n_cur, false))) return rc;
  HIPCHK(hipStreamSynchronize(C->stream));
  float ms = 0.f, t0 = 0.f;
  HIPCHK(hipEventElapsedTime(&ms, C->ev_k0, C->ev_k1));
  HIPCHK(hipEventElapsedTime(&t0, S->ev_t0, C->ev_k0));
  if (tail_whole) judge_order(S, C, n_cur, use, (double)ms);
  C->tail_iv.emplace_back(t0, t0 + ms);
  X.total_ms += ms;
  X.iters += C->h_counters[1];
  if (S->tune.trace)
    fprintf(stderr, "[loikb] tail launch: %6d instances on %u workgroups  %8.3f ms  inst-iters %9u (%.1f M/s)"
                    "  wave-iters %7u H-rebuild %3.0f%%\n",
            n, grid.x, ms, C->h_counters[1], C->h_counters[1] / ms / 1e3,
            C->h_counters[5], 100.0 * C->h_counters[6] / (C->h_counters[5] ? C->h_counters[5] : 1));
  C->stats.launches++; C->stats.tail_launches++;
  return LOIKB_OK;
}

template <typename T>
int run_tail(loikb_solver_impl* S, Chunk* C, Params<T>& P, int cur, int n_cur, int n_live, double* ms_out,
             unsigned long long* iters_out, bool whole_set = false)
{
  loikb_solver_impl::Set& A = C->set[cur];
  const int nw = (n_cur + WAVE - 1) / WAVE;
  const bool flat_here = flat_applicable(S) && (P.mode & MODE_CACHE_H);
  const bool flat_1pw = one_per_wave(flat_kind(S));
  const bool small_flat = whole_set && cur == 0 && S->chunks.size() == 1 && flat_1pw && flat_here && n_cur <= S->tune.flat_small_batch &&
                          n_cur >= std::max(1, S->tune.flat_min_batch);
  if (whole_set && !small_flat) {
    hipLaunchKernelGGL(k_list_iota, grid1(n_cur), dim3(256), 0, C->stream, C->d_slots, n_cur);
  } else if (!whole_set) {
    C->h_wave.resize(2 * (size_t)nw + 2);
    int* cnt = C->h_wave.data();
    int* off = cnt + nw + 1;
    HIPCHK(hipMemcpyAsync(cnt, A.wave_live, sizeof(int) * nw, hipMemcpyDeviceToHost, C->stream));
    HIPCHK(hipStreamSynchronize(C->stream));
    int total = 0;
    for (int w = 0; w < nw; ++w) { off[w] = total; total += cnt[w]; }
    if (total != n_live) { g_last_error = "tail: live count mismatch"; return LOIKB_ERR_STATE; }
    HIPCHK(hipMemcpyAsync(A.wave_off, off, sizeof(int) * nw, hipMemcpyHostToDevice, C->stream));
    hipLaunchKernelGGL(k_list_live<T>, dim3(nw), dim3(WAVE), 0, C->stream, A.tiles, S->L, n_cur, A.wave_off, C->d_slots);
  }
  HIPCHK(hipGetLastError());
  const int G = lanes_per_instance(S);
  TailCtx<T> X{S, C, P, make_bufs<T>(S, C, cur), A, cur, n_cur, whole_set, small_flat, G, WAVE / G, S->plan.ndec, S->plan.kexp_lo, C->d_slots, n_live};
  P.B = n_cur;
  int tw = S->tune.tail_waves;
  while (tw > 1 && tw * tail_lds_bytes<T>(S->nc, G) > 160 * 1024) --tw;
  const size_t lds = tw * tail_lds_bytes<T>(S->nc, G);
  if (lds > 160 * 1024) { g_last_error = "tail kernel: constraint data exceeds the LDS of a CU"; return LOIKB_ERR_ARG; }
  if (lds > 64 * 1024) {
    HIPCHK(hipFuncSetAttribute((const void*)k_tail<T, true>, hipFuncAttributeMaxDynamicSharedMemorySize, (int)lds));
    HIPCHK(hipFuncSetAttribute((const void*)k_tail<T, false>, hipFuncAttributeMaxDynamicSharedMemorySize, (int)lds));
  }
  if (S->tune.lean_adapt && S->seen_hi >= S->seen_lo && !(S->opt.flags & LOIKB_OPT_FIXED_ITERS) && !S->opt.logging) {
    const int lo = std::max(X.kexp_lo, S->seen_lo - 1), hi = std::min(X.kexp_lo + X.ndec - 1, S->seen_hi + 1);
    if (hi >= lo) { X.kexp_lo = lo; X.ndec = hi - lo + 1; }
  }
  int rc = LOIKB_OK;
  bool engine_ran = true;
  if (flat_here && X.n >= (flat_1pw ? std::max(1, S->tune.flat_min_batch) : 64)) rc = launch_flat(X);
  else if (S->plan.lean && (P.mode & MODE_CACHE_H) && X.n >= 64) rc = launch_lean(X);
  else engine_ran = false;
  if (rc) return rc;
  if (!(engine_ran && X.n == 0) && (rc = launch_tail_kernel(X, tw, lds))) return rc;
  *ms_out = X.total_ms;
  *iters_out = X.iters;
  return LOIKB_OK;
}

template <typename T>
int run_chunk(loikb_solver_impl* S, Chunk* C)
{
  Params<T> P = make_params<T>(S);
  C->stats = loikb_stats{};
  C->unfinished_counted = false;
  C->small_finished = false;
  C->solve_iv.clear();
  C->tail_iv.clear();
  double kernel_ms = 0.0;
  const int max_total = S->opt.max_iter + 1;
  const bool can_compact = !(S->opt.flags & LOIKB_OPT_NO_COMPACTION) && !(S->opt.flags & LOIKB_OPT_FIXED_ITERS);
  const int compact_min = S->opt.compact_min_instances > 0 ? S->opt.compact_min_instances : 64 * WAVE;
  const double compact_ratio = S->tune.compact_ratio;
  const bool use_tail = can_compact && S->nb <= WAVE && S->opt.tail_max_instances >= 0;
  const double share = (double)C->B / (double)S->B;
  const int tail_max = std::max(1, (int)(batch_tail_max(S) * share));
  const bool trace = S->tune.trace;
  const int team_max = S->tune.team_max;
  auto edge_entries = [](const loikb_solver_impl::TeamSched& sc) {
    return std::max(std::max(sc.nslots, 1) * EDGE_ENT, sc.nw > 1 ? sc.nw * Norms<T>::NALL : 0);
  };
  auto lds_bytes = [&](const loikb_solver_impl::TeamSched& sc) {
    return (size_t)(edge_entries(sc) + std::max(sc.nvslots, 1) * 6) * WAVE * sizeof(T);
  };
  constexpr size_t LDS_CU = 160 * 1024, LDS_DEFAULT = 64 * 1024;
  const bool team_ok = S->sched[1].nw > 1 && lds_bytes(S->sched[1]) <= LDS_CU &&
                       5 * (S->sched[1].T_up + S->sched[1].T_down) <= 4 * (S->sched[0].T_up + S->sched[0].T_down);
  if (S->plan.solve_ok) {
    const size_t need = std::max(lds_bytes(S->sched[0]), team_ok ? lds_bytes(S->sched[1]) : (size_t)0);
    if (need > LDS_DEFAULT) {
      HIPCHK(hipFuncSetAttribute((const void*)k_solve<T, true, true>, hipFuncAttributeMaxDynamicSharedMemorySize, (int)need));
      HIPCHK(hipFuncSetAttribute((const void*)k_solve<T, false, true>, hipFuncAttributeMaxDynamicSharedMemorySize, (int)need));
      HIPCHK(hipFuncSetAttribute((const void*)k_solve<T, true, false>, hipFuncAttributeMaxDynamicSharedMemorySize, (int)need));
      HIPCHK(hipFuncSetAttribute((const void*)k_solve<T, false, false>, hipFuncAttributeMaxDynamicSharedMemorySize, (int)need));
    }
  }
  int cur = 0, n_cur = C->B;
  int done_iters = 0;
  unsigned long long inst_iters = 0;
  unsigned int n_live = 0;
  const bool direct_tail = direct_tail_of(S, C->B, tail_max);
  if (!S->plan.solve_ok && !direct_tail) {
    g_last_error = "internal: a tree too bushy for k_solve's LDS slots reached the streaming engine"; return LOIKB_ERR_STATE;
  }
  if (direct_tail) {
    double tms = 0.0;
    unsigned long long tit = 0;
    int rc = run_tail<T>(S, C, P, 0, C->B, C->B, &tms, &tit, true);
    if (rc) return rc;
    kernel_ms += tms;
    if (trace) fprintf(stderr, "[loikb] tail kernel from the first iteration: %d instances  %8.3f ms  inst-iters %9llu\n", C->B, tms, tit);
    C->stats.tail_ms = tms;
    C->stats.tail_instances = C->B;
    C->stats.tail_instance_iterations = tit;
    inst_iters = tit;
  }
  while (!direct_tail) {
    const int tiles_cur = (n_cur + WAVE - 1) / WAVE;
    const bool latency_bound = S->opt.compact_min_instances <= 0 && tiles_cur * (int)S->chunks.size() <= S->ncu;
    const bool may_compact_later = can_compact && n_cur > compact_min && !latency_bound;
    const int lat_iters = S->tune.lat_iters;
    int launch_iters = S->opt.max_launch_iters > 0 ? S->opt.max_launch_iters
                       : (may_compact_later ? 8 : (use_tail || (can_compact && n_cur > compact_min)) ? lat_iters : max_total);
    if (launch_iters > max_total - done_iters) launch_iters = max_total - done_iters;
    P.B = n_cur;
    P.max_launch_iters = launch_iters;
    Bufs<T> Bf = make_bufs<T>(S, C, cur);
    const loikb_solver_impl::TeamSched& sc = S->sched[(team_ok && n_cur <= team_max) ? 1 : 0];
    C->stats.team = sc.nw;
    const int edge_ent = edge_entries(sc);
    const Team tm{sc.d_up, sc.d_down, sc.d_rlist, sc.T_up, sc.T_down, edge_ent};
    const size_t lds = lds_bytes(sc);
    const dim3 grid((unsigned)((n_cur + WAVE - 1) / WAVE)), block(WAVE * sc.nw);
    HIPCHK(hipMemsetAsync(C->d_counters, 0, NCOUNTERS * sizeof(unsigned int), C->stream));
    HIPCHK(hipEventRecord(C->ev_k0, C->stream));
    if (sc.nw > 1) {
      if (S->href_diag) hipLaunchKernelGGL((k_solve<T, true, true>), grid, block, lds, C->stream, P, Bf, tm.up, tm.down, tm.rlist, tm.T_up, tm.T_down, tm.edge_ent);
      else hipLaunchKernelGGL((k_solve<T, false, true>), grid, block, lds, C->stream, P, Bf, tm.up, tm.down, tm.rlist, tm.T_up, tm.T_down, tm.edge_ent);
    } else {
      if (S->href_diag) hipLaunchKernelGGL((k_solve<T, true, false>), grid, block, lds, C->stream, P, Bf, tm.up, tm.down, tm.rlist, tm.T_up, tm.T_down, tm.edge_ent);
      else hipLaunchKernelGGL((k_solve<T, false, false>), grid, block, lds, C->stream, P, Bf, tm.up, tm.down, tm.rlist, tm.T_up, tm.T_down, tm.edge_ent);
    }
    HIPCHK(hipGetLastError());
    HIPCHK(hipEventRecord(C->ev_k1, C->stream));
    HIPCHK(hipMemcpyAsync(C->h_counters, C->d_counters, NCOUNTERS * sizeof(unsigned int), hipMemcpyDeviceToHost, C->stream));
    HIPCHK(hipStreamSynchronize(C->stream));
    float ms = 0.f, t0 = 0.f;
    HIPCHK(hipEventElapsedTime(&ms, C->ev_k0, C->ev_k1));
    HIPCHK(hipEventElapsedTime(&t0, S->ev_t0, C->ev_k0));
    C->solve_iv.emplace_back(t0, t0 + ms);
    kernel_ms += ms;
    C->stats.launches++;
    inst_iters += C->h_counters[1];
    n_live = C->h_counters[0];
    done_iters += launch_iters;
    if (trace)
      fprintf(stderr, "[loikb] launch %3d: set %d slots %7d iters %4d..%4d  %8.3f ms  inst-iters %9u (%.1f M/s)  live after %7u"
                      "  tile-iters %6u H-rebuild %3.0f%% fused %3.0f%%\n",
              C->stats.launches, cur, n_cur, done_iters - launch_iters + 1, done_iters, ms, C->h_counters[1],
              C->h_counters[1] / ms / 1e3, n_live, C->h_counters[2],
              100.0 * C->h_counters[3] / (C->h_counters[2] ? C->h_counters[2] : 1),
              100.0 * C->h_counters[4] / (C->h_counters[2] ? C->h_counters[2] : 1));
    if (n_live == 0 || done_iters >= max_total) break;
    if (use_tail && (int)n_live <= tail_max) {
      double tms = 0.0;
      unsigned long long tit = 0;
      int rc = run_tail<T>(S, C, P, cur, n_cur, (int)n_live, &tms, &tit);
      if (rc) return rc;
      kernel_ms += tms;
      if (trace) fprintf(stderr, "[loikb] tail kernel: %u instances  %8.3f ms  inst-iters %9llu\n", n_live, tms, tit);
      C->stats.tail_ms = tms;
      C->stats.tail_instances = (int)n_live;
      C->stats.tail_instance_iterations = tit;
      inst_iters += tit;
      n_live = 0;
      break;
    }
    if (may_compact_later && (double)n_live <= compact_ratio * n_cur) {
      const int dst = cur == 1 ? 2 : 1;
      int n_new = 0;
      int rc = compact<T>(S, C, cur, dst, n_cur, &n_new);
      if (rc) return rc;
      cur = dst;
      n_cur = n_new;
      C->stats.compactions++;
    }
  }
  if (cur != 0) {
    int rc = compact<T>(S, C, cur, -1, n_cur, nullptr);
    if (rc) return rc;
  }
  HIPCHK(hipStreamSynchronize(C->stream));
  C->stats.instance_iterations = inst_iters;
  if (!C->unfinished_counted) C->stats.n_unfinished = (int)n_live;
  C->stats.kernel_ms = kernel_ms;
  return LOIKB_OK;
}

template <typename T>
int run_main_loop_t(loikb_solver_impl* S)
{
  S->stats = loikb_stats{};
  ++S->solve_serial;
  S->stats.bytes_per_instance_iteration = (double)sizeof(T) * (203.0 * S->nb + 108.0 * S->nc);
  HIPCHK(hipEventRecord(S->ev_t0, S->stream));
  const int nchunks = (int)S->chunks.size();
  if (nchunks == 1) {
    Chunk* C = &S->chunks[0];
    C->stream = S->stream;
    int rc = run_chunk<T>(S, C);
    if (rc) return rc;
  } else {
    HIPCHK(hipEventRecord(S->ev_fork, S->stream));
    for (Chunk& C : S->chunks) HIPCHK(hipStreamWaitEvent(C.stream, S->ev_fork, 0));
    std::vector<std::thread> th;
    for (Chunk& C : S->chunks)
      th.emplace_back([S, &C]() {
        if (hipSetDevice(S->device) != hipSuccess) { C.rc = LOIKB_ERR_HIP; C.err = "hipSetDevice failed in a chunk thread"; return; }
        C.rc = run_chunk<T>(S, &C);
        if (C.rc) C.err = g_last_error;
      });
    for (auto& t : th) t.join();
    for (Chunk& C : S->chunks)
      if (C.rc) { g_last_error = C.err; return C.rc; }
  }
  Chunk* C0 = &S->chunks[0];
  const bool counted = nchunks == 1 && C0->unfinished_counted;
  if (!counted) {
    HIPCHK(hipMemsetAsync(C0->d_counters, 0, sizeof(unsigned int), S->stream));
    hipLaunchKernelGGL(k_count_unfinished<T>, grid1(S->B), dim3(256), 0, S->stream, S->home.tiles, S->L, S->B, C0->d_counters);
    HIPCHK(hipGetLastError());
    HIPCHK(hipMemcpyAsync(C0->h_counters, C0->d_counters, sizeof(unsigned int), hipMemcpyDeviceToHost, S->stream));
  }
  float tms = 0.f;
  if (counted && C0->small_finished) {
    HIPCHK(hipEventElapsedTime(&tms, S->ev_t0, C0->ev_k1));
  } else {
    HIPCHK(hipEventRecord(S->ev_t1, S->stream));
    HIPCHK(hipStreamSynchronize(S->stream));
    HIPCHK(hipEventElapsedTime(&tms, S->ev_t0, S->ev_t1));
  }
  S->stats.n_unfinished = counted ? C0->stats.n_unfinished : (int)C0->h_counters[0];
  for (const Chunk& C : S->chunks) {
    S->stats.instance_iterations += C.stats.instance_iterations;
    S->stats.launches += C.stats.launches;
    S->stats.compactions += C.stats.compactions;
    S->stats.tail_instances += C.stats.tail_instances;
    S->stats.tail_ms += C.stats.tail_ms;
    S->stats.kernel_ms += C.stats.kernel_ms;
    S->stats.tail_instance_iterations += C.stats.tail_instance_iterations;
    S->stats.tail_launches += C.stats.tail_launches;
    S->stats.lean_launches += C.stats.lean_launches;
    S->stats.flat_launches += C.stats.flat_launches;
    S->stats.flat_split_launches += C.stats.flat_split_launches;
    S->stats.flat_ordered += C.stats.flat_ordered;
    S->stats.flat_built += C.stats.flat_built;
    S->stats.queue_dry_ms += C.stats.queue_dry_ms;
    S->stats.lean_escaped += C.stats.lean_escaped;
    S->stats.hslots_ms += C.stats.hslots_ms;
    S->stats.lean_requeues += C.stats.lean_requeues;
    S->stats.team = C.stats.team;
  }
  S->stats.chunks = nchunks;
  S->stats.total_ms = tms;
  auto busy = [&](bool tail) {
    std::vector<std::pair<float, float>> iv;
    for (const Chunk& C : S->chunks) {
      const auto& v = tail ? C.tail_iv : C.solve_iv;
      iv.insert(iv.end(), v.begin(), v.end());
    }
    std::sort(iv.begin(), iv.end());
    double tot = 0.0;
    float lo = 0.f, hi = -1.f;
    for (const auto& x : iv) {
      if (hi < lo || x.first > hi) { if (hi >= lo) tot += hi - lo; lo = x.first; hi = x.second; }
      else if (x.second > hi) hi = x.second;
    }
    if (hi >= lo) tot += hi - lo;
    return tot;
  };
  S->stats.solve_busy_ms = busy(false);
  S->stats.tail_busy_ms = busy(true);
  return LOIKB_OK;
}


int run_pass_solve(loikb_solver_impl* S, bool logged);
static int start_mu(loikb_solver_impl* S)
{
  if (S->opt.mu_update_strat != LOIKB_MU_MAXEIGENVALUE) return LOIKB_OK;
  const double mu = spectral_mu0(S);
  if (mu != S->mu_start) { S->seen_lo = 1 << 20; S->seen_hi = -(1 << 20); S->end_hist_n = 0; }
  S->mu_start = mu;
  return reset_home(S, RS_MU);
}

int run_main_loop(loikb_solver_impl* S)
{
  struct QueueOffer { loikb_solver_impl* S; ~QueueOffer() { for (loikb_solver_impl::Chunk& C : S->chunks) C.queue_ready = false; } } offer{S};
  S->pass_active = false;
  if (S->opt.mu_update_strat != LOIKB_MU_DEFAULT && S->opt.mu_update_strat != LOIKB_MU_OSQP &&
      S->opt.mu_update_strat != LOIKB_MU_MAXEIGENVALUE && !(S->opt.flags & LOIKB_OPT_FIXED_ITERS)) {
    g_last_error = "[FirstOrderLoikOptimizedTpl::UpdateMu]: mu update strategy not supported";
    return LOIKB_ERR_MU_STRATEGY;
  }
  int rc;
  if (!S->plan.solve_ok && !bushy_goes_on_chip(S)) rc = run_pass_solve(S, false);
  else if ((rc = start_mu(S))) {}
  else rc = S->f32 ? run_main_loop_t<float>(S) : run_main_loop_t<double>(S);
  return rc;
}

template <typename T>
__global__ void k_limi(char* tiles, Layout L, const JointDesc* __restrict__ jd, const int* __restrict__ sel,
                       const int* __restrict__ last, int nsel, int B, double* __restrict__ out)
{
  const int b = blockIdx.x * blockDim.x + threadIdx.x;
  if (b >= B) return;
  char* lp = lane_ptr<T>(tiles, L, b);
  for (int e = 0; e < nsel; ++e) {
    double Ra[9] = {1, 0, 0, 0, 1, 0, 0, 0, 1}, ta[3] = {0, 0, 0};
    for (int i = sel[e] + 1; i <= last[e] + 1; ++i) {
      T R[9], t[3];
      const char* rec = lp + (size_t)(i - 1) * JREC * pair_bytes<T>();
      const typename Vec2<T>::type cs = ldp<T>(rec, JP_CS);
      joint_xform<T>(jd[i], rec, cs.x, cs.y, R, t);
      double Rn[9], tn[3];
      for (int r = 0; r < 3; ++r) {
        for (int c = 0; c < 3; ++c) Rn[3 * r + c] = Ra[3 * r] * (double)R[c] + Ra[3 * r + 1] * (double)R[3 + c] + Ra[3 * r + 2] * (double)R[6 + c];
        tn[r] = ta[r] + Ra[3 * r] * (double)t[0] + Ra[3 * r + 1] * (double)t[1] + Ra[3 * r + 2] * (double)t[2];
      }
      for (int k = 0; k < 9; ++k) Ra[k] = Rn[k];
      for (int k = 0; k < 3; ++k) ta[k] = tn[k];
    }
    double* o = out + ((size_t)b * nsel + e) * 12;
    for (int k = 0; k < 9; ++k) o[k] = Ra[k];
    for (int k = 0; k < 3; ++k) o[9 + k] = ta[k];
  }
}

template <typename T>
__global__ void k_residual_vecs(char* tiles, Layout L, const JointDesc* __restrict__ jd, const T* __restrict__ uni,
                                const double* __restrict__ href_tab, int a_shared, const int* __restrict__ sel, int nl, int B, int dual,
                                double* __restrict__ out)
{
  const int b = blockIdx.x * blockDim.x + threadIdx.x;
  if (b >= B) return;
  char* lp = lane_ptr<T>(tiles, L, b);
  double* o = out + (size_t)b * (6 * nl + L.nb);
  for (int e = 0; e < nl; ++e) {
    const int i = sel[e] + 1;
    const char* rec = lp + (size_t)(i - 1) * JREC * pair_bytes<T>();
    T v[6];
    ld6<T>(rec, JP_V, v);
    if (dual) {
      T g[6];
      ld6<T>(rec, JP_G, g);
      const double* row = href_tab + (size_t)i * HREF_ROW;
      for (int r = 0; r < 6; ++r) {
        double a = 0.0;
        for (int k = 0; k < 6; ++k) a += row[6 * r + k] * (double)v[k];
        o[6 * e + r] = a - row[36 + r] + (double)g[r];
      }
    } else {
      const int cs = jd[i].cslot;
      for (int r = 0; r < 6; ++r) o[6 * e + r] = 0.0;
      if (cs >= 0) {
        const char* crec = lp + (size_t)(L.off_c + cs * L.crec) * pair_bytes<T>();
        T bb[6];
        ld6<T>(crec, CP_B, bb);
        for (int r = 0; r < 6; ++r) {
          double a = 0.0;
          for (int k = 0; k < 6; ++k) {
            const int q = 6 * r + k;
            const T A = a_shared ? uni[cs * 36 + q] : *elem_ptr<T>(const_cast<char*>(crec), CP_A + q / 2, q & 1);
            a += (double)A * (double)v[k];
          }
          o[6 * e + r] = a - (double)bb[r];
        }
      }
    }
  }
  for (int j = 0; j < L.nb; ++j) {
    const char* rec = lp + (size_t)j * JREC * pair_bytes<T>();
    const typename Vec2<T>::type nus = ldp<T>(rec, JP_NUS);
    o[6 * nl + j] = dual ? (double)nus.y : (double)nus.x - (double)ldp<T>(rec, JP_WZ).y;
  }
}

__global__ void k_select_rows(const double* __restrict__ src, int nrow_src, int w, const int* __restrict__ sel, int nsel,
                              int B, double* __restrict__ dst)
{
  const int b = blockIdx.x * blockDim.x + threadIdx.x;
  if (b >= B) return;
  for (int e = 0; e < nsel; ++e)
    for (int k = 0; k < w; ++k) dst[((size_t)b * nsel + e) * w + k] = src[((size_t)b * nrow_src + sel[e]) * w + k];
}

}

struct loikb_solver : loikb_solver_impl {};

extern "C" {

int loikb_version(void) { return LOIKB_VERSION; }

int loikb_sweep_schedule(const int* parents, int njoints, int team, int direction, int steps_cap, int* joint_out,
                         int* flags_out, int* slot_out, int* lds_slots_out)
{
  if (!parents || njoints < 2 || team < 1 || team > MAX_TEAM || (direction != 0 && direction != 1) || !joint_out)
    return LOIKB_ERR_ARG;
  for (int i = 1; i < njoints; ++i)
    if (parents[i] < 0 || parents[i] >= i) return LOIKB_ERR_ARG;
  loikb_solver_impl::TeamSched sc;
  build_team_schedule(std::vector<int>(parents, parents + njoints), team, sc);
  const int T = direction == 0 ? sc.T_up : sc.T_down;
  const std::vector<StepDesc>& st = direction == 0 ? sc.up : sc.down;
  if (T > steps_cap) return LOIKB_ERR_ARG;
  for (int w = 0; w < team; ++w)
    for (int t = 0; t < steps_cap; ++t) {
      const bool in = t < T;
      joint_out[w * steps_cap + t] = in ? st[(size_t)w * T + t].joint : 0;
      if (flags_out) flags_out[w * steps_cap + t] = in ? st[(size_t)w * T + t].flags : 0;
      if (slot_out) slot_out[w * steps_cap + t] = in && (st[(size_t)w * T + t].flags & SF_OUT_LDS) ? st[(size_t)w * T + t].wslot : -1;
    }
  if (lds_slots_out) *lds_slots_out = direction == 0 ? sc.nslots : sc.nvslots;
  return T;
}

int loikb_flat_schedule(const int* parents, int njoints, int* out, int cap, int* meta)
{
  if (!parents || njoints < 2 || !meta) return LOIKB_ERR_ARG;
  for (int i = 1; i < njoints; ++i)
    if (parents[i] < 0 || parents[i] >= i) { g_last_error = "parents[i] must be < i"; return LOIKB_ERR_MODEL; }
  loikb_solver_impl::FlatSched fs;
  build_flat_schedule(std::vector<int>(parents, parents + njoints), fs);
  meta[0] = fs.ok; meta[1] = fs.G; meta[2] = fs.nanc; meta[3] = fs.nscan; meta[4] = fs.njmp;
  if (!fs.ok) { g_last_error = fs.why; return LOIKB_OK; }
  constexpr int W = (int)(sizeof(FlatLane) / sizeof(int));
  static_assert(sizeof(FlatLane) == sizeof(int) * (2 + FLAT_JMP + FLAT_MAXA + FLAT_RED + 1 + FLAT_PART), "FlatLane is a plain int record");
  if (!out || cap < fs.G * W) return fs.G * W;
  memcpy(out, fs.lanes.data(), sizeof(FlatLane) * fs.lanes.size());
  for (int l = 0; l < fs.G; ++l) out[l * W + (int)(offsetof(FlatLane, helper) / sizeof(int))] &= 1;
  return LOIKB_OK;
}

int loikb_flat_variant(int kind, int hm, int sliced, int logging, int mur, int* out4)
{
  if ((kind != 1 && kind != 2) || hm < 0 || hm > 3 || mur < 0 || mur > 2 || !out4) return LOIKB_ERR_ARG;
  const FlatVariant v = flat_variant(kind == 2 ? FlatKind::Flat2 : FlatKind::Flat1, hm, sliced != 0, logging != 0, mur);
  out4[0] = v.sliced; out4[1] = v.hm; out4[2] = v.log; out4[3] = v.mur;
  return LOIKB_OK;
}

const char* loikb_last_error(void) { return g_last_error.c_str(); }

const char* loikb_status_string(int code)
{
  switch (code) {
  case LOIKB_OK: return "ok";
// ... 60 lines not shown
    return LOIKB_ERR_NO_DEVICE;
  }
  auto fail = [&](int code) { loikb_destroy(S); return code; };
#define TRY(x) do { int _rc = (x); if (_rc) return fail(_rc); } while (0)
#define HIPTRY(x) do { hipError_t _e = (x); if (_e != hipSuccess) { g_last_error = std::string(#x) + ": " + hipGetErrorString(_e); return fail(LOIKB_ERR_HIP); } } while (0)
  HIPTRY(hipSetDevice(S->device));
  {
    hipDeviceProp_t prop;
    if (hipGetDeviceProperties(&prop, S->device) == hipSuccess && prop.multiProcessorCount > 0) S->ncu = prop.multiProcessorCount;
  }
  if (opts->flags & LOIKB_OPT_OWN_STREAM) {
    HIPTRY(hipStreamCreateWithFlags(&S->own_stream, hipStreamNonBlocking));
    S->stream = S->own_stream;
  }
  HIPTRY(hipEventCreate(&S->ev_t0));
  HIPTRY(hipEventCreate(&S->ev_t1));
  HIPTRY(hipEventCreate(&S->ev_fork));
  void* tmp = nullptr;
  TRY(alloc_dev(S, &tmp, sizeof(JointDesc) * S->nj)); S->d_jd = (JointDesc*)tmp;
  TRY(alloc_dev(S, &tmp, sizeof(int) * S->nj)); S->d_idx_q = (int*)tmp;
  TRY(alloc_dev(S, &tmp, sizeof(int) * ROWMAP_CAP)); S->d_rowmap = (int*)tmp;
  TRY(alloc_dev(S, &tmp, sizeof(double) * (size_t)S->B * S->nq)); S->d_q = (double*)tmp;
  TRY(alloc_dev(S, &tmp, sizeof(TailTopo) * S->nj)); S->d_topo = (TailTopo*)tmp;
  TRY(alloc_dev(S, &tmp, sizeof(int) * (S->child_list.size() + 1))); S->d_child_list = (int*)tmp;
  HIPTRY(hipMemcpyAsync(S->d_topo, S->topo.data(), sizeof(TailTopo) * S->nj, hipMemcpyHostToDevice, S->stream));
  if (!S->child_list.empty())
    HIPTRY(hipMemcpyAsync(S->d_child_list, S->child_list.data(), sizeof(int) * S->child_list.size(),
                          hipMemcpyHostToDevice, S->stream));
  TRY(alloc_dev(S, &S->d_uni, S->esz * ((size_t)(S->nc > 0 ? S->nc : 1) * 57 + 2 * (size_t)S->nb)));
  HIPTRY(hipMemcpyAsync(S->d_idx_q, S->idx_q.data(), sizeof(int) * S->nj, hipMemcpyHostToDevice, S->stream));
  {
    std::vector<int> sel(S->ext_nj), fsel(S->ext_nj);
    for (int i = 1; i < S->ext_nj; ++i) { sel[i - 1] = S->link_of[i] - 1; fsel[i - 1] = S->first_of[i] - 1; }
    TRY(alloc_dev(S, &tmp, sizeof(int) * S->ext_nj)); S->d_link_sel = (int*)tmp;
    TRY(alloc_dev(S, &tmp, sizeof(int) * S->ext_nj)); S->d_first_sel = (int*)tmp;
    HIPTRY(hipMemcpyAsync(S->d_link_sel, sel.data(), sizeof(int) * (S->ext_nj - 1), hipMemcpyHostToDevice, S->stream));
    HIPTRY(hipMemcpyAsync(S->d_first_sel, fsel.data(), sizeof(int) * (S->ext_nj - 1), hipMemcpyHostToDevice, S->stream));
    HIPTRY(hipStreamSynchronize(S->stream));
  }
  for (auto& sc : S->sched) {
    TRY(alloc_dev(S, &tmp, sizeof(StepDesc) * sc.up.size())); sc.d_up = (StepDesc*)tmp;
    TRY(alloc_dev(S, &tmp, sizeof(StepDesc) * sc.down.size())); sc.d_down = (StepDesc*)tmp;
    TRY(alloc_dev(S, &tmp, sizeof(int) * sc.rlist.size())); sc.d_rlist = (int*)tmp;
    HIPTRY(hipMemcpyAsync(sc.d_rlist, sc.rlist.data(), sizeof(int) * sc.rlist.size(), hipMemcpyHostToDevice, S->stream));
  }
  if (S->flat.ok) {
    TRY(alloc_dev(S, &tmp, sizeof(FlatLane) * S->flat.lanes.size())); S->flat.d_lanes = (FlatLane*)tmp;
    HIPTRY(hipMemcpyAsync(S->flat.d_lanes, S->flat.lanes.data(), sizeof(FlatLane) * S->flat.lanes.size(), hipMemcpyHostToDevice, S->stream));
  }
  TRY(upload_jd(S));
  TRY(ensure_layout(S, true));
  HIPTRY(hipStreamSynchronize(S->stream));
#undef TRY
#undef HIPTRY
  *out = S;
  return LOIKB_OK;
}

int loikb_destroy(loikb_solver* S)
{
  if (!S) return LOIKB_OK;
  (void)hipSetDevice(S->device);
  destroy_chunks(S);
  const hipStream_t own_stream = S->own_stream;
  const hipEvent_t ev[3] = {S->ev_fork, S->ev_t0, S->ev_t1};
  delete S;
  if (own_stream) (void)hipStreamDestroy(own_stream);
  for (hipEvent_t e : ev) if (e) (void)hipEventDestroy(e);
  (void)hipGetLastError();
  return LOIKB_OK;
}

int loikb_set_stream(loikb_solver* S, void* hip_stream)
{
  if (!S) return LOIKB_ERR_ARG;
  S->stream = (hipStream_t)hip_stream;
  return LOIKB_OK;
}

static int solve_init_impl(loikb_solver* S, const double* q, const double* H_ref, const double* v_ref, const int* c_ids,
                           int nc, const double* Ais, const double* bis, const double* lb, const double* ub, int nbound,
                           int in_flags, bool final_sync)
{
  if (!S || !q || !H_ref || !v_ref || (nc > 0 && (!c_ids || !Ais || !bis)) || !lb || !ub) return LOIKB_ERR_ARG;
  HIPCHK(hipSetDevice(S->device));
  int rc;
  if ((rc = validate_problem(S, H_ref, c_ids, nc, nbound))) return rc;
  S->pose.have_tasks = false;
  memcpy(S->Href, H_ref, 36 * sizeof(double));
  S->href_known = true;
  S->per_link = false;
  if ((rc = ensure_layout(S, in_flags & LOIKB_A_SHARED))) return rc;
  S->pass_active = false;
  struct Deferred { loikb_solver_impl* S; bool armed; ~Deferred() { if (armed) (void)flush_uni(S); S->defer_sync = false; if (armed) (void)hipStreamSynchronize(S->stream); } } deferred{S, true};
  S->defer_sync = true;
  S->pin_off = 0;
  if ((rc = reset_home(S, RS_SOLVER | (S->opt.warm_start ? 0 : RS_DATA_COLD)))) return rc;
  if ((rc = set_problem(S, H_ref, v_ref, c_ids, nc, Ais, bis, lb, ub, nbound, in_flags))) return rc;
  if ((rc = fwd_pass_init(S, q, in_flags))) return rc;
  if ((rc = flush_uni(S))) return rc;
  S->defer_sync = false;
  deferred.armed = false;
  if (final_sync) HIPCHK(hipStreamSynchronize(S->stream));
  return LOIKB_OK;
}

int loikb_solve_init(loikb_solver* S, const double* q, const double* H_ref, const double* v_ref, const int* c_ids,
                     int nc, const double* Ais, const double* bis, const double* lb, const double* ub, int nbound,
                     int in_flags)
{
  return solve_init_impl(S, q, H_ref, v_ref, c_ids, nc, Ais, bis, lb, ub, nbound, in_flags, true);
}

int loikb_update_references(loikb_solver* S, const double* H_refs, const double* v_refs, int n)
{
  if (!S || !H_refs || !v_refs) return LOIKB_ERR_ARG;
  if (!S->have_problem) { g_last_error = "UpdateReferences() before SolveInit()"; return LOIKB_ERR_STATE; }
  if (n != S->ext_nj) { g_last_error = "'H_refs', 'v_refs' have wrong size (one entry per joint incl. the universe)"; return LOIKB_ERR_REFS_SIZE; }
  for (int e = 1; e < n; ++e)
    if (!symmetric6(H_refs + 36 * e)) { g_last_error = "H_refs[i] must be symmetric"; return LOIKB_ERR_HREF_NOT_SYMMETRIC; }
  HIPCHK(hipSetDevice(S->device));
  HIPCHK(hipStreamSynchronize(S->stream));
  ++S->inputs_epoch;
  fill_href_tab(S, H_refs, v_refs, 36, 6);
  S->tab_bcast = false;
  S->href_diag = true;
  for (int e = 0; e < n; ++e) {
    const double *He = H_refs + 36 * e, *ve = v_refs + 6 * e;
    for (int i = 0; i < 6; ++i) {
      double a = 0.0;
      for (int k = 0; k < 6; ++k) {
        a += He[6 * i + k] * ve[k];
        if (e > 0 && i != k && He[6 * i + k] != 0.0) S->href_diag = false;
      }
      if (std::fabs(a) > S->Hv_inf_norm) S->Hv_inf_norm = std::fabs(a);
    }
  }
  S->per_link = true;
  S->pass_active = false;
  int rc;
  if ((rc = upload_href_tab(S))) return rc;
  if ((rc = ensure_hslots(S))) return rc;
  return reset_home(S, RS_HCACHE);
}

static int run_logged(loikb_solver_impl* S, int redo_reset = 0);

int loikb_solve(loikb_solver* S)
{
  if (!S) return LOIKB_ERR_ARG;
  if (!S->have_problem) { g_last_error = "Solve() before SolveInit()"; return LOIKB_ERR_STATE; }
  HIPCHK(hipSetDevice(S->device));
  int rc;
  if ((rc = reset_home(S, RS_RECURSION | RS_SOLVER, !S->opt.logging))) return rc;
  return S->opt.logging ? run_logged(S, RS_RECURSION | RS_SOLVER) : run_main_loop(S);
}

int loikb_solve_full(loikb_solver* S, const double* q, const double* H_ref, const double* v_ref, const int* c_ids,
                     int nc, const double* Ais, const double* bis, const double* lb, const double* ub, int nbound,
                     int in_flags)
{
  if (!S) return LOIKB_ERR_ARG;
  S->offer_queue = !S->opt.logging;
  int rc = solve_init_impl(S, q, H_ref, v_ref, c_ids, nc, Ais, bis, lb, ub, nbound, in_flags, false);
  S->offer_queue = false;
  if (rc) { for (loikb_solver_impl::Chunk& C : S->chunks) C.queue_ready = false; return rc; }
  rc = S->opt.logging ? run_logged(S, S->opt.warm_start ? 0 : (RS_SOLVER | RS_DATA_COLD | RS_Y | RS_HCACHE)) : run_main_loop(S);
  if (rc) (void)hipStreamSynchronize(S->stream);
  return rc;
}

int loikb_solve_tailored(loikb_solver* S, const double* q, int c_id, const double* Ai, const double* bi, int in_flags)
{
  if (!S || (c_id >= 0 && (!Ai || !bi))) return LOIKB_ERR_ARG;
  if (!S->have_problem) { g_last_error = "tailored Solve() before SolveInit()"; return LOIKB_ERR_STATE; }
  HIPCHK(hipSetDevice(S->device));
  int rc;
  struct Deferred { loikb_solver_impl* S; bool armed; ~Deferred() { if (armed) (void)flush_uni(S); S->defer_sync = false; if (armed) (void)hipStreamSynchronize(S->stream); } } deferred{S, true};
  S->defer_sync = true;
  S->pin_off = 0;
  if ((rc = reset_home(S, RS_SOLVER | (S->opt.warm_start ? 0 : RS_DATA_COLD)))) return rc;
  if (c_id >= 0 && (rc = update_eq_single(S, c_id, Ai, bi, in_flags))) return rc;
  S->offer_queue = !S->opt.logging;
  rc = fwd_pass_init(S, q, in_flags);
  S->offer_queue = false;
  if (rc == LOIKB_OK) rc = flush_uni(S);
  if (rc) { for (loikb_solver_impl::Chunk& C : S->chunks) C.queue_ready = false; return rc; }
  S->defer_sync = false;
  deferred.armed = false;
  return S->opt.logging ? run_logged(S, S->opt.warm_start ? 0 : (RS_SOLVER | RS_DATA_COLD | RS_Y | RS_HCACHE)) : run_main_loop(S);
}

int loikb_update_eq_constraint(loikb_solver* S, int c_id, const double* Ai, const double* bi, int in_flags)
{
  if (!S || !bi) return LOIKB_ERR_ARG;
  if (!S->have_problem) { g_last_error = "UpdateEqConstraint() before SolveInit()"; return LOIKB_ERR_STATE; }
  HIPCHK(hipSetDevice(S->device));
  int rc;
  if ((rc = update_eq_single(S, c_id, Ai, bi, in_flags))) return rc;
  S->pass_active = false;
  return reset_home(S, RS_HCACHE);
}

int loikb_update_ineq_constraints(loikb_solver* S, const double* lb, const double* ub, int nbound, int in_flags)
{
  if (!S || !lb || !ub) return LOIKB_ERR_ARG;
  if (!S->have_problem) { g_last_error = "UpdateIneqConstraints() before SolveInit()"; return LOIKB_ERR_STATE; }
  if (nbound != S->nv) { g_last_error = "lb/ub dimension differs from model.nv"; return LOIKB_ERR_INEQ_DIM; }
  HIPCHK(hipSetDevice(S->device));
  ++S->inputs_epoch;
  S->pass_active = false;
  int rc;
  if ((rc = update_ineq(S, lb, ub, in_flags))) { (void)hipStreamSynchronize(S->stream); return rc; }
  HIPCHK(hipStreamSynchronize(S->stream));
  return LOIKB_OK;
}

int loikb_add_eq_constraint(loikb_solver* S, int c_id, const double* Ai, const double* bi, int in_flags)
{
  if (!S || !Ai || !bi) return LOIKB_ERR_ARG;
  if (!S->have_problem) { g_last_error = "AddEqConstraint() before SolveInit()"; return LOIKB_ERR_STATE; }
  for (int c = 0; c < S->nc_active; ++c)
    if (S->active_ids[c] == c_id) return loikb_update_eq_constraint(S, c_id, Ai, bi, in_flags);
  if (c_id < 1 || c_id >= S->ext_nj) { g_last_error = "constraint link id out of range"; return LOIKB_ERR_ARG; }
  if (S->nc_active >= S->nc) {
    g_last_error = "AddEqConstraint: no free constraint slot (loikb_options.eq_c_capacity)";
    return LOIKB_ERR_EQ_C_SIZE;
  }
  HIPCHK(hipSetDevice(S->device));
  ++S->inputs_epoch;
  S->pose.have_tasks = false;
  int rc;
  const int k = S->nc_active;
  if ((rc = null_constraint_slots(S, k, k + 1))) return rc;
  S->active_ids.push_back(c_id);
  ++S->nc_active;
  if ((rc = bind_constraint_slots(S))) return rc;
  if ((rc = update_eq_single(S, c_id, Ai, bi, in_flags))) {
    S->active_ids.pop_back();
    --S->nc_active;
    (void)bind_constraint_slots(S);
    return rc;
  }
  return reset_home(S, RS_HCACHE);
}

int loikb_remove_eq_constraint(loikb_solver* S, int c_id)
{
  if (!S) return LOIKB_ERR_ARG;
  if (!S->have_problem) { g_last_error = "RemoveEqConstraint() before SolveInit()"; return LOIKB_ERR_STATE; }
  int found = -1;
  for (int c = 0; c < S->nc_active; ++c)
    if (S->active_ids[c] == c_id) { found = c; break; }
  if (found < 0) {
    g_last_error = "WARNING RemoveEqConstraint: no constraint defined at link id, nothing to remove";
    return LOIKB_NOTHING_TO_REMOVE;
  }
  HIPCHK(hipSetDevice(S->device));
  ++S->inputs_epoch;
  S->pose.have_tasks = false;
  int rc;
  if ((rc = edit_constraints(S, found, S->nc_active, 1))) return rc;
  for (int c = found; c + 1 < S->nc_active; ++c) {
    memcpy(S->A_host.data() + 36 * c, S->A_host.data() + 36 * (c + 1), 36 * sizeof(double));
    if (S->a_shared && (rc = upload_shared_A(S, S->A_host.data() + 36 * c, c))) return rc;
  }
  const double zero[36] = {0};
  memset(S->A_host.data() + 36 * (S->nc_active - 1), 0, 36 * sizeof(double));
  if ((rc = upload_shared_A(S, zero, S->nc_active - 1))) return rc;
  S->active_ids.erase(S->active_ids.begin() + found);
  --S->nc_active;
  if ((rc = bind_constraint_slots(S))) return rc;
  if ((rc = constraint_products(S, 0, S->nc, false))) return rc;
  return reset_home(S, RS_HCACHE);
}

int loikb_num_eq_c(const loikb_solver* S) { return S ? S->nc_active : 0; }
int loikb_eq_c_capacity(const loikb_solver* S) { return S ? S->nc : 0; }
int loikb_active_constraint_ids(const loikb_solver* S, int* out, int cap)
{
  if (!S || (cap > 0 && !out)) return LOIKB_ERR_ARG;
  for (int c = 0; c < S->nc_active && c < cap; ++c) out[c] = S->active_ids[c];
  return S->nc_active;
}

int loikb_integrate(loikb_solver* S, double dt)
{
  if (!S) return LOIKB_ERR_ARG;
  if (!S->have_q) { g_last_error = "integrate: no configurations resident on the device yet"; return LOIKB_ERR_STATE; }
  ++S->inputs_epoch;
  HIPCHK(hipSetDevice(S->device));
  with_real(S, [&](auto t) {
    hipLaunchKernelGGL(k_advance_q<decltype(t)>, grid1(S->B), dim3(256), 0, S->stream, S->d_q, (const double*)nullptr, 0, S->nq,
                       S->d_jd, S->d_idx_q, S->L, S->B, S->home.tiles, dt);
  });
  HIPCHK(hipGetLastError());
  return LOIKB_OK;
}

int loikb_synchronize(loikb_solver* S)
{
  if (!S) return LOIKB_ERR_ARG;
  HIPCHK(hipSetDevice(S->device));
  HIPCHK(hipDeviceSynchronize());
  return LOIKB_OK;
}
// ... 533 lines not shown
                          to_dev ? hipMemcpyDeviceToDevice : hipMemcpyDeviceToHost, S->stream));
    HIPCHK(hipStreamSynchronize(S->stream));
    return LOIKB_OK;
  }
  const Layout& L = S->L;
  const int nb = S->nb;
  const int nl = S->ext_nj - 1;
  std::vector<int> rm;
  bool is_int = false;
  int mask = 0;
  auto per_joint = [&](int pair, int half) { for (int j = 0; j < nb; ++j) rm.push_back((j * JREC + pair) * 2 + half); };
  auto per_joint_vec = [&](int pair, int n) {
    for (int i = 1; i <= nl; ++i)
      for (int k = 0; k < n; ++k) rm.push_back(((S->link_of[i] - 1) * JREC + pair + k / 2) * 2 + (k & 1));
  };
  auto per_constraint_vec = [&](int pair) {
    for (int c = 0; c < S->nc_active; ++c)
      for (int k = 0; k < 6; ++k) rm.push_back((L.off_c + c * L.crec + pair + k / 2) * 2 + (k & 1));
  };
  switch (field) {
  case LOIKB_F_Z: case LOIKB_F_NU: case LOIKB_F_W: case LOIKB_F_VIS: case LOIKB_F_FIS: case LOIKB_F_YIS: result_rows(S, field, rm); break;
  case LOIKB_F_STF_PLUS_W: per_joint(JP_NUS, 1); break;
  case LOIKB_F_R: per_joint(JP_R, 0); break;
  case LOIKB_F_DINV: per_joint(JP_R, 1); break;
  case LOIKB_F_G: per_joint_vec(JP_G, 6); break;
  case LOIKB_F_PIS: break;
  case LOIKB_F_UDINV:
    for (int j = 0; j < nb; ++j)
      for (int k = 0; k < 6; ++k) rm.push_back((j * JREC + JP_UD + k / 2) * 2 + (k & 1));
    break;
  case LOIKB_F_HIS: break;

  case LOIKB_F_ATY: per_constraint_vec(CP_ATY); break;
  case LOIKB_F_LIMI: break;
  case LOIKB_F_PRIMAL_RESIDUAL_VEC: case LOIKB_F_DUAL_RESIDUAL_VEC: break;
  case LOIKB_F_ITER: is_int = true; rm.push_back((L.off_s + SP_BI) * 2 + 1); break;
  case LOIKB_F_STATUS: is_int = true; mask = -(ST_CONVERGED | ST_PRIMAL_INF | ST_TAIL | ST_DONE); rm.push_back((L.off_s + SP_ST) * 2); break;
  case LOIKB_F_CONVERGED: is_int = true; mask = ST_CONVERGED; rm.push_back((L.off_s + SP_ST) * 2); break;
  case LOIKB_F_PRIMAL_INFEASIBLE: is_int = true; mask = ST_PRIMAL_INF; rm.push_back((L.off_s + SP_ST) * 2); break;
  case LOIKB_F_MU: rm.push_back((L.off_s + SP_MU) * 2); break;
  case LOIKB_F_MU_UPDATES: is_int = true; rm.push_back((L.off_s + SP_FLIP) * 2); break;
  default:
    static_assert(LOIKB_F_TAIL_SOLVE_ITER - LOIKB_F_PRIMAL_RESIDUAL + 1 == NSCAL, "scalar field ids out of sync");
    if (field >= LOIKB_F_PRIMAL_RESIDUAL && field <= LOIKB_F_TAIL_SOLVE_ITER) {
      const int idx = field - LOIKB_F_PRIMAL_RESIDUAL;
      rm.push_back((L.off_s + SP_SCAL + idx / 2) * 2 + (idx & 1));
    } else {
      return LOIKB_ERR_ARG;
    }
  }
  const bool resvec = field == LOIKB_F_PRIMAL_RESIDUAL_VEC || field == LOIKB_F_DUAL_RESIDUAL_VEC;
  const int n = field == LOIKB_F_LIMI ? 12 * nl : field == LOIKB_F_HIS ? 21 * nl : field == LOIKB_F_PIS ? 6 * nl
                : resvec ? 6 * nl + nb : (int)rm.size();
  const bool select = nl != nb && (field == LOIKB_F_HIS || field == LOIKB_F_PIS);
  double* final_dst = nullptr;
  void* d_tmp = nullptr;
  const size_t bytes = (is_int ? sizeof(int) : sizeof(double)) * (size_t)S->B * n;
  double* dst = (double*)out;
  int rc;
  if (!to_dev) {
    if ((rc = regrow(S->d_stage, bytes))) return rc;
    dst = S->d_stage.as<double>();
  }
  if (select) {
    final_dst = dst;
    if ((rc = regrow(S->d_getscr[0], sizeof(double) * (size_t)S->B * nb * (field == LOIKB_F_HIS ? 21 : 6)))) return rc;
    d_tmp = S->d_getscr[0];
    dst = (double*)d_tmp;
  }
  if ((field == LOIKB_F_UDINV || field == LOIKB_F_PIS) && S->ud_stale) {
    if ((rc = regrow(S->d_getscr[1], S->esz * (size_t)S->B * nb * 21))) return rc;
    void* d_scr = S->d_getscr[1];
    with_real(S, [&](auto t) {
      using T = decltype(t);
      hipLaunchKernelGGL(k_rebuild_ud<T>, grid1(S->B), dim3(256), 0, S->stream, S->home.tiles, L, (const JointDesc*)S->d_jd,
                         (const T*)S->d_uni, (T)S->opt.rho, (T)S->opt.mu_equality_scale_factor, (const T*)S->d_href,
                         (int)S->a_shared, S->B, (T*)d_scr);
    });
    HIPCHK(hipGetLastError());
    HIPCHK(hipStreamSynchronize(S->stream));
    S->ud_stale = false;
  }
  if (field == LOIKB_F_HIS) {
    with_real(S, [&](auto t) {
      using T = decltype(t);
      hipLaunchKernelGGL(k_rebuild_his<T>, grid1(S->B), dim3(256), 0, S->stream, S->home.tiles, L, S->d_jd, (const T*)S->d_uni,
                         (T)S->opt.rho, (T)S->opt.mu_equality_scale_factor, (const T*)S->d_href, (int)S->a_shared, S->B, dst);
    });
  } else if (field == LOIKB_F_PIS) {
    with_real(S, [&](auto t) {
      hipLaunchKernelGGL(k_rebuild_pis<decltype(t)>, grid1(S->B), dim3(256), 0, S->stream, S->home.tiles, L, S->d_jd, S->B, dst);
    });
  } else if (resvec) {
    const int dual = field == LOIKB_F_DUAL_RESIDUAL_VEC;
    with_real(S, [&](auto t) {
      using T = decltype(t);
      hipLaunchKernelGGL(k_residual_vecs<T>, grid1(S->B), dim3(256), 0, S->stream, S->home.tiles, L, S->d_jd, (const T*)S->d_uni,
                         S->d_href64, (int)S->a_shared, S->d_link_sel, nl, S->B, dual, dst);
    });
  } else if (field == LOIKB_F_LIMI) {
    with_real(S, [&](auto t) {
      hipLaunchKernelGGL(k_limi<decltype(t)>, grid1(S->B), dim3(256), 0, S->stream, S->home.tiles, L, S->d_jd, S->d_first_sel, S->d_link_sel, nl, S->B, dst);
    });
  } else {
    if ((rc = set_rowmap(S, rm))) return rc;
    const size_t dbytes = sizeof(double) * (size_t)S->B * (size_t)n;
    if (!to_dev && n > 0 && dbytes <= ((size_t)256 << 10)) {
      if (dbytes > S->h_res.bytes()) {
        if (S->h_res) HIPCHK(hipStreamSynchronize(S->stream));
        BUFCHK(S->h_res.regrow((size_t)256 << 10));
      }
      const long long total = (long long)S->B * n;
      const dim3 g((unsigned)((total + 255) / 256));
      with_real(S, [&](auto t) {
        hipLaunchKernelGGL(k_download_elems<decltype(t)>, g, dim3(256), 0, S->stream, S->home.tiles, L, (const int*)S->d_rowmap, n, S->B, S->h_res);
      });
      HIPCHK(hipGetLastError());
      HIPCHK(hipStreamSynchronize(S->stream));
      if (is_int) {
        int* o = (int*)out;
        for (long long i = 0; i < total; ++i) {
          const int v = (int)S->h_res[i];
          o[i] = mask > 0 ? ((v & mask) ? 1 : 0) : (mask < 0 ? (v & -mask) : v);
        }
      } else {
        memcpy(out, S->h_res, dbytes);
      }
      return LOIKB_OK;
    }
    with_real(S, [&](auto t) {
      hipLaunchKernelGGL(k_download_rows<decltype(t)>, grid1(S->B), dim3(256), 0, S->stream, S->home.tiles, L, S->d_rowmap, n,
                         S->B, dst, (int)is_int, mask);
    });
  }
  HIPCHK(hipGetLastError());
  if (select) {
    hipLaunchKernelGGL(k_select_rows, grid1(S->B), dim3(256), 0, S->stream, (const double*)d_tmp, nb,
                       field == LOIKB_F_HIS ? 21 : 6, S->d_link_sel, nl, S->B, final_dst);
    HIPCHK(hipGetLastError());
    dst = final_dst;
  }
  if (!to_dev) HIPCHK(hipMemcpyAsync(out, dst, bytes, hipMemcpyDeviceToHost, S->stream));
  HIPCHK(hipStreamSynchronize(S->stream));
  return LOIKB_OK;
}

int loikb_debug_device_memory(unsigned long long out[4])
{
  if (!out) return LOIKB_ERR_ARG;
  for (int k = 0; k < 4; ++k) out[k] = g_devmem[k].load();
  return LOIKB_OK;
}

#ifdef LOIKB_TAIL_PROF
int loikb_debug_wave_dbg(unsigned long long* out)
{
  HIPCHK(hipMemcpyFromSymbol(out, HIP_SYMBOL(loikb::g_wave_dbg), sizeof(unsigned long long) * 4096 * 6));
  return LOIKB_OK;
}
int loikb_debug_tail_prof(unsigned long long* out)
{
  HIPCHK(hipMemcpyFromSymbol(out, HIP_SYMBOL(loikb::g_tail_prof), sizeof(unsigned long long) * 32));
#ifdef LOIKB_FLAT_SEPARATE_TU
  unsigned long long f[32];
  if (loikb_flat_prof_read(f, 0, 0)) return LOIKB_ERR_HIP;
  if (f[8]) memcpy(out, f, sizeof(f));
#endif
  return LOIKB_OK;
}
int loikb_debug_tail_prof_all(unsigned long long* out, int reset)
{
  HIPCHK(hipMemcpyFromSymbol(out, HIP_SYMBOL(loikb::g_tail_prof_all), sizeof(unsigned long long) * 32));
  if (reset) {
    unsigned long long z[32] = {0};
    HIPCHK(hipMemcpyToSymbol(HIP_SYMBOL(loikb::g_tail_prof_all), z, sizeof(z)));
  }
#ifdef LOIKB_FLAT_SEPARATE_TU
  unsigned long long f[32];
  if (loikb_flat_prof_read(f, 1, reset)) return LOIKB_ERR_HIP;
  for (int k = 0; k < 32; ++k) out[k] += f[k];
#endif
  return LOIKB_OK;
}
#endif

}

#include "loik_host_pose.hpp"
```

### loik_amd/csrc/loik_lean.hpp

```cpp
#pragma once

#include "loik_tail.hpp"

namespace loikb {

constexpr int LXS = 14;
constexpr int LXA = 0, LXB = 6;
constexpr int LHS = 21;
constexpr int HSLOT_PAIRS = 11;
enum : int { IS_MU = 0, IS_KEXP, IS_ITER, IS_STATUS, IS_TAILIT, IS_C1, IS_C2, IS_NFLIP, IS_TOLP, IS_TOLD, IS_DYQP, IS_ATDY,
             IS_UBP, IS_LBM, IS_BNORM, IS_PRIMAL, IS_DUAL, IS_PRT, IS_PRS, IS_DUALV, IS_STF, IS_DX, IS_DZ, IS_DFIS,
             IS_DYIS, IS_DW, IS_DVIS, IS_DNU, IS_AV, IS_NU, IS_HREFV, IS_G, IS_TGIN, IS_STY, IS_MULAST,
             IS_RED , ISC = IS_RED + 12 };

constexpr int LCD = 26, LCA = 36;
constexpr int LEAN_Q_HEAD = 7, LEAN_Q_TAIL = 8, LEAN_Q_REQUEUES = 9, LEAN_Q_RETIRED = 10;
constexpr int LEAN_DECADES_SEEN = 11;
constexpr int NCOUNTERS = 96;
constexpr int ORDER_DEC_HIST = 64;
enum : int { LC_PAD = 0, LC_B = 1, LC_ATB = 7, LC_Y = 13, LC_ATY = 19 };

template <typename T>
#ifdef LOIKB_PLAIN_RECORDS
__device__ __forceinline__ T cld(const char* p) { return *reinterpret_cast<const T*>(p); }
// ... 651 lines not shown
      load_instance(fetch_plain());
#endif
    }
    TAIL_TP(7)
  }
#ifdef LOIKB_TAIL_PROF
  if (blockIdx.x == 0 && threadIdx.x == 0) {
    for (int k = 0; k < 8; ++k) g_tail_prof[k] = prof_[k];
    for (int k = 8; k < 12; ++k) g_tail_prof[2 + k] = prof_[k];
    g_tail_prof[8] = n_wave_iters;
    g_tail_prof[9] = (clock64() - clk0_) * 100000ull / (wall_clock64() - wall0_ + 1);
  }
  if (lane == 0) {
    const int wid = blockIdx.x * TAIL_WAVES + wv;
    if (wid < 4096) {
      g_wave_dbg[wid][0] = wall0_; g_wave_dbg[wid][1] = dbg_last_; g_wave_dbg[wid][2] = wall_clock64();
      g_wave_dbg[wid][3] = n_wave_iters; g_wave_dbg[wid][4] = dbg_both_; g_wave_dbg[wid][5] = dbg_sw_;
    }
  }
#endif
  if (lane == 0) {
    atomicAdd(&Bf.counters[5], n_wave_iters);
  }
  if (jlane == 0) {
    atomicAdd(&Bf.counters[6], n_slot_loads >> 16);
    atomicOr(&Bf.counters[LEAN_DECADES_SEEN], n_slot_loads & 0xFFFFu);
  }
}

template <typename T, bool HDIAG, bool PERLINK = false>
__global__ void __launch_bounds__(WAVE)
k_hslots(const Params<T> P, const Bufs<T> Bf, const JointDesc* __restrict__ jd, const TailTopo* __restrict__ topo,
         const int* __restrict__ child_list, int maxdepth, int maxchild, const int* __restrict__ slots, int nslots, int G,
         T* __restrict__ hslots, int kexp_lo, int ndec)
{
  extern __shared__ __attribute__((aligned(16))) unsigned char smem_raw[];
  const Layout& L = P.L;
  T* xch = reinterpret_cast<T*>(smem_raw);
  constexpr int HX = 22;
  const int lane = threadIdx.x & (WAVE - 1);
  const int ipw = WAVE / G;
  const int sub = lane / G, jlane = lane % G, gbase = sub * G;
  const int idx = blockIdx.x * ipw + sub;
  const bool has_inst = idx < nslots;
  const bool isj = has_inst && jlane < L.nb;
  const int jl = jlane < L.nb ? jlane : 0;
  const JointDesc d = jd[jl + 1];
  const TailTopo tp = topo[jl + 1];
  const int depth = jlane < L.nb ? tp.depth : 0;
  const bool rev = d.flags & JF_REVOLUTE;
  const T mass = (d.flags & JF_MASSLESS) ? T(0) : T(1);
  const T* const hrow = PERLINK ? P.href_tab + (size_t)(jl + 1) * HREF_ROW : nullptr;
  const bool has_parent = !(d.flags & JF_PARENT_ROOT);
  const T ax0 = (T)d.axis[0], ax1 = (T)d.axis[1], ax2 = (T)d.axis[2];
  const int slot = slots[has_inst ? idx : 0];
  const int sidx = slot;
  char* ip = lane_ptr<T>(Bf.tiles, L, slot);
  const char* rec = ip + (size_t)jl * JREC * pair_bytes<T>();
  T R[9], t[3];
  {
    const typename Vec2<T>::type cs = ldp<T>(rec, JP_CS);
    joint_xform<T>(d, rec, cs.x, cs.y, R, t);
  }
  T ata[21];
#pragma unroll
  for (int k = 0; k < 21; ++k) ata[k] = T(0);
  if (isj && d.cslot >= 0) {
    const char* crec = ip + (size_t)(L.off_c + d.cslot * L.crec) * pair_bytes<T>();
    for (int k = 0; k < 21; ++k)
      ata[k] = (P.mode & MODE_A_SHARED) ? Bf.uni[L.nc * 36 + d.cslot * 21 + k]
                                        : *reinterpret_cast<const T*>(crec + (size_t)(CP_ATA + k / 2) * pair_bytes<T>() + (k & 1) * sizeof(T));
  }
  typename Vec2<T>::type* hp = reinterpret_cast<typename Vec2<T>::type*>(hslots);
  T mu = P.mu0;
  for (int k = 0; k < kexp_lo; ++k) mu *= T(10);
  for (int k = 0; k > kexp_lo; --k) mu *= T(0.1);
  const int lag = maxdepth - depth;
  for (int st = 0; st < maxdepth + ndec - 1; ++st) {
    const int dsl = st - lag;
    const bool on = isj && depth > 0 && dsl >= 0 && dsl < ndec;
    T part[21];
#pragma unroll
    for (int k = 0; k < 21; ++k) part[k] = T(0);
    if (on) {
      const T mu_eq = P.mu_scale * mu, mu_in = mu;
      T hh[21];
#pragma unroll
      for (int a = 0; a < 6; ++a)
#pragma unroll
        for (int b2 = a; b2 < 6; ++b2)
          hh[sym(a, b2)] = mass * ((a == b2 ? P.rho : T(0)) + ((HDIAG && a != b2) ? T(0) : (PERLINK ? hrow[6 * a + b2] : P.Href[6 * a + b2])));
#pragma unroll
      for (int k = 0; k < 21; ++k) hh[k] += mu_eq * ata[k];
      for (int c = 0; c < tp.nchild; ++c) {
        const T* x = xch + (gbase + child_list[tp.child_start + c]) * HX;
#pragma unroll
        for (int k = 0; k < 21; ++k) hh[k] += x[k];
      }
      T U[6], UD[6];
      T dinv;
      if (rev) {
#pragma unroll
        for (int k = 0; k < 6; ++k) U[k] = hh[sym(k, 3)] * ax0 + hh[sym(k, 4)] * ax1 + hh[sym(k, 5)] * ax2;
        dinv = T(1) / ((ax0 * U[3] + ax1 * U[4] + ax2 * U[5]) + mu_in);
      } else {
#pragma unroll
        for (int k = 0; k < 6; ++k) U[k] = hh[sym(k, 0)] * ax0 + hh[sym(k, 1)] * ax1 + hh[sym(k, 2)] * ax2;
        dinv = T(1) / ((ax0 * U[0] + ax1 * U[1] + ax2 * U[2]) + mu_in);
      }
      if (d.flags & JF_HELICAL) {
        const T ph = (T)d.pitch;
#pragma unroll
        for (int k = 0; k < 6; ++k) U[k] += ph * (hh[sym(k, 0)] * ax0 + hh[sym(k, 1)] * ax1 + hh[sym(k, 2)] * ax2);
        dinv = T(1) / (((ax0 * U[3] + ax1 * U[4] + ax2 * U[5]) + ph * (ax0 * U[0] + ax1 * U[1] + ax2 * U[2])) + mu_in);
      }
#pragma unroll
      for (int k = 0; k < 6; ++k) UD[k] = U[k] * dinv;
#pragma unroll
      for (int k = 0; k < 10; ++k) hp[hslot_pair(sidx, ndec, dsl, G, k, jlane)] = typename Vec2<T>::type{hh[2 * k], hh[2 * k + 1]};
      hp[hslot_pair(sidx, ndec, dsl, G, 10, jlane)] = typename Vec2<T>::type{hh[20], dinv};
      if (has_parent) {
#pragma unroll
        for (int a = 0; a < 6; ++a)
#pragma unroll
          for (int b2 = a; b2 < 6; ++b2) hh[sym(a, b2)] -= UD[a] * U[b2];
        congr_sym(R, t, hh, part);
      }
      mu *= T(10);
    }
    tail_sync();
    if (on && has_parent) {
      T* x = xch + lane * HX;
#pragma unroll
      for (int k = 0; k < 21; ++k) x[k] = part[k];
    }
    tail_sync();
  }
}

#ifndef LOIKB_FLAT_KERNELS_TU
__global__ void k_ring_fill(int* __restrict__ ring, int cap, const int* __restrict__ list, int n, unsigned int* __restrict__ counters)
{
  const int i = blockIdx.x * blockDim.x + threadIdx.x;
  if (i < cap) ring[i] = i < n ? list[i] : -1;
  if (i == 0) {
    counters[LEAN_Q_HEAD] = 0u; counters[LEAN_Q_TAIL] = (unsigned int)n; counters[LEAN_Q_REQUEUES] = 0u;
    counters[LEAN_Q_RETIRED] = 0u;
    counters[14] = (unsigned int)wall_clock64();
  }
}
#endif

#ifndef LOIKB_FLAT_KERNELS_TU
__global__ void k_queue_init_iota(int* __restrict__ ring, int cap, int* __restrict__ list, int n, unsigned int* __restrict__ counters, int ncounters)
{
  const int i = blockIdx.x * blockDim.x + threadIdx.x;
  if (i < cap) ring[i] = i < n ? i : -1;
  if (i < n) list[i] = i;
  if (i < ncounters) {
    unsigned int v = 0u;
    if (i == LEAN_Q_TAIL) v = (unsigned int)n;
    if (i == 14) v = (unsigned int)wall_clock64();
    counters[i] = v;
  }
}
template <typename T>
__global__ void __launch_bounds__(WAVE) k_reset_and_queue(char* tiles, Layout L, int what, T mu0, int ntiles, int* __restrict__ ring, int cap,
                                                          int* __restrict__ list, int n, unsigned int* __restrict__ counters, int ncounters)
{
  if ((int)blockIdx.x < ntiles) { reset_tile<T>(tiles, L, what, mu0, (int)blockIdx.x, (int)threadIdx.x); return; }
  const int i = ((int)blockIdx.x - ntiles) * WAVE + (int)threadIdx.x;
  if (i < cap) ring[i] = i < n ? i : -1;
  if (i < n) list[i] = i;
  if (i < ncounters) {
    unsigned int v = 0u;
    if (i == LEAN_Q_TAIL) v = (unsigned int)n;
    if (i == 14) v = (unsigned int)wall_clock64();
    counters[i] = v;
  }
}
#endif

template <typename T>
__global__ void k_list_unfinished(char* tiles, Layout L, const int* __restrict__ list_in, int n_in, int* __restrict__ list_out,
                                  unsigned int* __restrict__ counter)
{
  const int i = blockIdx.x * blockDim.x + threadIdx.x;
  if (i >= n_in) return;
  const int b = list_in[i];
  char* sp = lane_ptr<T>(tiles, L, b);
  const int status = (int)ldp<T>(sp + (size_t)L.off_s * pair_bytes<T>(), SP_ST).x;
  if (!(status & ST_DONE)) list_out[atomicAdd(counter, 1u)] = b;
  if (!(status & (ST_CONVERGED | ST_PRIMAL_INF))) atomicAdd(counter + 1, 1u);
}

template <typename T>
__global__ void __launch_bounds__(256) k_small_finish(char* tiles, Layout L, const int* __restrict__ list_in, int n_in, int* __restrict__ list_out,
                                                      unsigned int* __restrict__ counters, int ncounters, unsigned int* __restrict__ host_counters)
{
  for (int i = threadIdx.x; i < n_in; i += blockDim.x) {
    const int b = list_in[i];
    char* sp = lane_ptr<T>(tiles, L, b);
    const int status = (int)ldp<T>(sp + (size_t)L.off_s * pair_bytes<T>(), SP_ST).x;
    if (!(status & ST_DONE)) list_out[atomicAdd(counters + 3, 1u)] = b;
    if (!(status & (ST_CONVERGED | ST_PRIMAL_INF))) atomicAdd(counters + 4, 1u);
  }
  __threadfence();
  __syncthreads();
  for (int k = threadIdx.x; k < ncounters; k += blockDim.x)
    host_counters[k] = __hip_atomic_load(counters + k, __ATOMIC_RELAXED, __HIP_MEMORY_SCOPE_AGENT);
}

constexpr int ORDER_BINS = 256;
template <typename T>
__device__ __forceinline__ int order_bin(char* tiles, const Layout& L, int b, int max_iter)
{
  char* sp = lane_ptr<T>(tiles, L, b);
  const int it = (int)ldp<T>(sp + (size_t)L.off_s * pair_bytes<T>(), SP_BI).y;
  const int k = (int)(((long long)it * ORDER_BINS) / (max_iter > 0 ? max_iter : 1));
  return ORDER_BINS - 1 - (k < 0 ? 0 : k > ORDER_BINS - 1 ? ORDER_BINS - 1 : k);
}
template <typename T>
__global__ void __launch_bounds__(256) k_order_count(char* tiles, Layout L, int n, int max_iter, unsigned int* __restrict__ bins,
                                                     unsigned int* __restrict__ dec_hist = nullptr)
{
  __shared__ unsigned int h[ORDER_BINS], hd[32];
  h[threadIdx.x] = 0u;
  if (threadIdx.x < 32) hd[threadIdx.x] = 0u;
  __syncthreads();
  const int b = blockIdx.x * blockDim.x + threadIdx.x;
  if (b < n) {
    atomicAdd(&h[order_bin<T>(tiles, L, b, max_iter)], 1u);
    if (dec_hist != nullptr) {
      const int kx = (int)ldp<T>(lane_ptr<T>(tiles, L, b) + (size_t)L.off_s * pair_bytes<T>(), SP_MU).y;
      atomicAdd(&hd[kx < -16 ? 0 : kx > 15 ? 31 : kx + 16], 1u);
    }
  }
  __syncthreads();
  if (h[threadIdx.x]) atomicAdd(&bins[threadIdx.x], h[threadIdx.x]);
  if (dec_hist != nullptr && threadIdx.x < 32 && hd[threadIdx.x]) atomicAdd(&dec_hist[threadIdx.x], hd[threadIdx.x]);
}
#ifndef LOIKB_FLAT_KERNELS_TU
__global__ void __launch_bounds__(ORDER_BINS) k_order_scan(unsigned int* __restrict__ bins)
{
  __shared__ unsigned int h[ORDER_BINS];
  const int t = threadIdx.x;
  h[t] = bins[t];
  __syncthreads();
  for (int d = 1; d < ORDER_BINS; d <<= 1) {
    const unsigned int v = t >= d ? h[t - d] : 0u;
    __syncthreads();
    h[t] += v;
    __syncthreads();
  }
  bins[ORDER_BINS + t] = h[t] - bins[t];
}
#endif
template <typename T>
__global__ void __launch_bounds__(256) k_order_scatter(char* tiles, Layout L, int n, int max_iter, unsigned int* __restrict__ bins,
                                                       int* __restrict__ order)
{
  __shared__ unsigned int h[ORDER_BINS], base[ORDER_BINS];
  h[threadIdx.x] = 0u;
  __syncthreads();
  const int b = blockIdx.x * blockDim.x + threadIdx.x;
  int bin = 0;
  unsigned int rank = 0u;
  if (b < n) { bin = order_bin<T>(tiles, L, b, max_iter); rank = atomicAdd(&h[bin], 1u); }
  __syncthreads();
  if (h[threadIdx.x]) base[threadIdx.x] = atomicAdd(&bins[ORDER_BINS + threadIdx.x], h[threadIdx.x]);
  __syncthreads();
  if (b < n) order[base[bin] + rank] = b;
}

}
```

Before: 7.165 million.

## Skip reset pass via virtual reset and fuse queue/order setup kernels in flat engine

Adds a virtual-reset route: instead of launching a reset pass over all tiles before each solve, the flat prep kernel synthesizes the zeroed solver scalars (mu set to mu0, others zero) and skips loading y/aty constraint vectors. The reset is deferred and flushed on every other path. It also fuses list iota, ring fill, order copy and bin clearing into one queue-init kernel, and merges the unfinished-list and order-count kernels into k_finish_order. The aim is to remove whole-batch memory passes and kernel launches per solve, at the cost of more complex state tracking and a deferred reset that must stay correct across paths.

```diff
diff --git a/loik_amd/csrc/loik_device.hpp b/loik_amd/csrc/loik_device.hpp
--- a/loik_amd/csrc/loik_device.hpp
+++ b/loik_amd/csrc/loik_device.hpp
@@ -77,6 +77,7 @@
   MODE_MU_OSQP = 16,
   MODE_ZERO_STATE = 32,
   MODE_FLAT_PREP = 64,
+  MODE_VIRTUAL_RESET = 128,
 };
 
 
diff --git a/loik_amd/csrc/loik_flat_prep.hpp b/loik_amd/csrc/loik_flat_prep.hpp
--- a/loik_amd/csrc/loik_flat_prep.hpp
+++ b/loik_amd/csrc/loik_flat_prep.hpp
@@ -54,7 +54,10 @@
     in.nus = ldp<T>(rec, JP_NUS);
     if (!(P.mode & MODE_BND_SHARED)) in.lu = ldp<T>(rec, JP_LBUB);
   }
-  if (jlane < PRS_N) {
+  const bool virt = (P.mode & MODE_VIRTUAL_RESET) != 0;
+  if (virt && jlane < PRS_N && jlane != PRS_BNORM && jlane != PRS_TGIN) {
+    in.sc = jlane == PRS_MU ? P.mu0 : T(0);
+  } else if (jlane < PRS_N) {
     const char* srec = ip + (size_t)L.off_s * pair_bytes<T>();
     const int sc_i = jlane == 3 ? SC_TOL_PRIMAL : jlane == 4 ? SC_TOL_DUAL : jlane == 5 ? SC_DELTA_Y_QP : jlane == 6 ? SC_AT_DELTA_Y_QP
                    : jlane == 7 ? SC_UB_DY_PLUS : jlane == 8 ? SC_LB_DY_MINUS : jlane == 9 ? SC_COND1 : jlane == 10 ? SC_COND2
@@ -69,7 +72,7 @@
   for (int c = 0; c < PREP_NC; ++c) {
     if (c >= L.nc) break;
     const char* crec = ip + (size_t)(L.off_c + c * L.crec) * pair_bytes<T>();
-    if (jlane < 18) {
+    if (jlane < (virt ? 6 : 18)) {
       const int which = jlane / 6, k = jlane % 6;
       const int pair = which == 0 ? CP_B : which == 1 ? CP_Y : CP_ATY;
       in.cv[c] = *reinterpret_cast<const T*>(crec + (size_t)(pair + k / 2) * pair_bytes<T>() + (k & 1) * sizeof(T));
diff --git a/loik_amd/csrc/loik_host.hip b/loik_amd/csrc/loik_host.hip
--- a/loik_amd/csrc/loik_host.hip
+++ b/loik_amd/csrc/loik_host.hip
@@ -120,6 +120,7 @@
   int small_finish = 1;
   int flat_slice = -1;
   bool flat_prep = true;
+  bool flat_seq = true;
   bool flat_zero_state = true;
   int flat_order_holdoff = 4;
   bool flat_order = true;
@@ -153,6 +154,7 @@
     if (const char* e = getenv("LOIKB_FLAT_ORDER")) flat_order = atoi(e) != 0;
     if (const char* e = getenv("LOIKB_FLAT_ZERO_STATE")) flat_zero_state = atoi(e) != 0;
     if (const char* e = getenv("LOIKB_FLAT_PREP")) flat_prep = atoi(e) != 0;
+    if (const char* e = getenv("LOIKB_FLAT_SEQ")) flat_seq = atoi(e) != 0;
     if (const char* e = getenv("LOIKB_FLAT_ORDER_HOLDOFF")) flat_order_holdoff = std::max(0, atoi(e));
     geti("LOIKB_TAIL_WAVES", tail_waves); tail_waves = std::max(1, std::min(TAIL_WAVES, tail_waves));
     geti("LOIKB_LEAN_DECADES", lean_decades); lean_decades = std::max(1, std::min(15, lean_decades));
@@ -310,6 +312,7 @@
   loikb_stats stats{};
   bool pass_active = false;
   bool zero_state = false;
+  int reset_pending = 0;
   unsigned long long inputs_epoch = 1;
   bool href_known = false;
   bool tab_bcast = false;
@@ -1033,6 +1036,14 @@
   return LOIKB_OK;
 }
 
+int flush_pending_reset(loikb_solver_impl* S)
+{
+  const int what = S->reset_pending;
+  if (!what) return LOIKB_OK;
+  S->reset_pending = 0;
+  return reset_home(S, what);
+}
+
 int to_device(loikb_solver_impl* S, const void* src, size_t bytes, bool src_device, const void** out)
 {
   if (src_device) { *out = src; return LOIKB_OK; }
@@ -1792,6 +1803,23 @@
   return direct_tail_of(S, S->B, std::max(1, batch_tail_max(S)));
 }
 
+static bool flat_prep_route(const loikb_solver_impl* S, const Chunk* C, int n)
+{
+  return flat_kind(S) == FlatKind::Flat2 && S->tune.flat_prep && !flat_any_mu(S) && !S->opt.logging && flat_prep_fits(S) &&
+         C->d_prep && (size_t)n * flat_prep_stride(S->nc) * sizeof(double) <= C->d_prep.bytes();
+}
+
+static bool virtual_reset_route(const loikb_solver_impl* S)
+{
+  if (!S->tune.flat_seq || S->chunks.size() != 1 || S->f32 || S->opt.logging || S->opt.max_iter < 2) return false;
+  if (S->opt.mu_update_strat != LOIKB_MU_DEFAULT) return false;
+  if (!S->tune.flat_zero_state || !flat_applicable(S) || (S->opt.flags & LOIKB_OPT_NO_H_CACHE)) return false;
+  if (!S->plan.solve_ok && !bushy_goes_on_chip(S)) return false;
+  if (!direct_tail_of(S, S->B, std::max(1, batch_tail_max(S)))) return false;
+  if (S->B <= S->tune.flat_small_batch || S->B < std::max(1, S->tune.flat_min_batch)) return false;
+  return flat_prep_route(S, &S->chunks[0], S->B);
+}
+
 template <typename T>
 struct TailCtx {
   loikb_solver_impl* S; Chunk* C; Params<T>& P; Bufs<T> Bf;
@@ -1802,26 +1830,29 @@
   const int* list; int n;
   double total_ms = 0.0;
   unsigned long long iters = 0;
+  bool list_pending = false;
 };
 
 struct OrderUse { bool ordered = false, was_stale = false; };
 
-static int take_up_order(const loikb_solver_impl* S, Chunk* C, bool eligible, bool count_down, int n_cur, OrderUse* use)
+static int take_up_order(const loikb_solver_impl* S, Chunk* C, bool eligible, bool count_down, int n_cur, OrderUse* use, bool copy = true)
 {
   use->ordered = eligible && order_usable(S, C, n_cur);
   use->was_stale = use->ordered && C->order_epoch != S->inputs_epoch;
   if (count_down && C->order_holdoff > 0) --C->order_holdoff;
-  if (use->ordered) HIPCHK(hipMemcpyAsync(C->d_slots, C->d_order, sizeof(int) * (size_t)n_cur, hipMemcpyDeviceToDevice, C->stream));
+  if (use->ordered && copy) HIPCHK(hipMemcpyAsync(C->d_slots, C->d_order, sizeof(int) * (size_t)n_cur, hipMemcpyDeviceToDevice, C->stream));
   C->stats.flat_ordered += use->ordered ? 1 : 0;
   return LOIKB_OK;
 }
 
 template <typename T>
-static int leave_order(const loikb_solver_impl* S, Chunk* C, const loikb_solver_impl::Set& A, int n_cur, bool flat_engine)
-{
-  HIPCHK(hipMemsetAsync(C->d_order_bins, 0, sizeof(unsigned int) * 2 * ORDER_BINS, C->stream));
-  hipLaunchKernelGGL(k_order_count<T>, grid1(n_cur), dim3(256), 0, C->stream, A.tiles, S->L, n_cur, S->opt.max_iter, C->d_order_bins,
-                     flat_engine ? C->d_counters + ORDER_DEC_HIST : (unsigned int*)nullptr);
+static int leave_order(const loikb_solver_impl* S, Chunk* C, const loikb_solver_impl::Set& A, int n_cur, bool flat_engine, bool counted = false)
+{
+  if (!counted) {
+    HIPCHK(hipMemsetAsync(C->d_order_bins, 0, sizeof(unsigned int) * 2 * ORDER_BINS, C->stream));
+    hipLaunchKernelGGL(k_order_count<T>, grid1(n_cur), dim3(256), 0, C->stream, A.tiles, S->L, n_cur, S->opt.max_iter, C->d_order_bins,
+                       flat_engine ? C->d_counters + ORDER_DEC_HIST : (unsigned int*)nullptr);
+  }
   if (flat_engine) HIPCHK(hipMemcpyAsync(C->h_counters, C->d_counters, NCOUNTERS * sizeof(unsigned int), hipMemcpyDeviceToHost, C->stream));
   hipLaunchKernelGGL(k_order_scan, dim3(1), dim3(ORDER_BINS), 0, C->stream, C->d_order_bins);
   hipLaunchKernelGGL(k_order_scatter<T>, grid1(n_cur), dim3(256), 0, C->stream, A.tiles, S->L, n_cur, S->opt.max_iter, C->d_order_bins, C->d_order);
@@ -1851,6 +1882,7 @@
   int ndec, kexp_lo, dw0, nw;
   int slice;
   bool prep;
+  bool virt;
   double cu_sh; dim3 grid;
 };
 
@@ -1942,7 +1974,7 @@
 }
 
 template <typename T>
-static int flat_read_back(TailCtx<T>& X, const FlatLaunch& F, OrderUse use, bool order_pass, bool small_finish, bool queue_ready, int* next)
+static int flat_read_back(TailCtx<T>& X, const FlatLaunch& F, OrderUse use, bool order_pass, bool small_finish, bool queue_ready, int* next, bool fused_queue)
 {
   loikb_solver_impl* S = X.S; Chunk* C = X.C;
   const int n_first = X.n, n_cur = X.n_cur;
@@ -1975,13 +2007,15 @@
   }
   C->stats.hslots_ms += hms;
   if (C->h_counters[FLAT_COUNTERS_DRY])
-    C->stats.queue_dry_ms += (double)(unsigned int)(C->h_counters[FLAT_COUNTERS_TDRY] - C->h_counters[FLAT_COUNTERS_T0]) * 1e-5;
+    C->stats.queue_dry_ms += (double)(unsigned int)(C->h_counters[FLAT_COUNTERS_TDRY] - C->h_counters[FLAT_COUNTERS_T0]) * 1e-5
+                             - (fused_queue ? (double)hms : 0.0);
   if (one_per_wave(F.kind) && X.whole_set && n_first == n_cur) judge_order(S, C, n_cur, use, (double)ms - (double)hms);
   if (S->tune.trace)
     fprintf(stderr, "[loikb] flat engine: %6d instances on %u workgroups, done at %8.3f ms (slots %6.3f ms)  "
                     "inst-iters %9u  wave-iters %7u  slot loads %7u (+ %u served from LDS)  escaped %u  still iterating %u%s\n",
             n_first, F.grid.x, ms, hms, C->h_counters[1], C->h_counters[5], C->h_counters[6],
-            C->h_counters[FLAT_COUNTERS_SLOT_HITS], escaped, C->h_counters[3], F.prep ? "  fresh instances from prepared records" : "");
+            C->h_counters[FLAT_COUNTERS_SLOT_HITS], escaped, C->h_counters[3],
+            F.virt ? "  fresh instances from prepared records, no reset pass" : F.prep ? "  fresh instances from prepared records" : "");
   C->stats.lean_escaped += (int)escaped;
   C->tail_iv.emplace_back(t0, t0 + ms);
   X.total_ms = ms; X.n = (int)C->h_counters[3]; X.list = next;
@@ -2012,50 +2046,66 @@
   if (whole_set && S->zero_state && S->tune.flat_zero_state) P.mode |= MODE_ZERO_STATE;
   const bool queue_ready = small_flat && C->queue_ready && n_cur == S->B;
   C->queue_ready = false;
-  if (!queue_ready && small_flat) hipLaunchKernelGGL(k_queue_init_iota, grid1(std::max(C->ring_cap, NCOUNTERS)), dim3(256), 0, C->stream, C->d_ring, C->ring_cap, C->d_slots, n_cur, C->d_counters, NCOUNTERS);
+  const bool fused_queue = X.list_pending && !small_flat && whole_set && X.list == C->d_slots && n == n_cur;
+  if (X.list_pending && !fused_queue) { g_last_error = "internal: the flat engine was left a list it cannot write"; return LOIKB_ERR_STATE; }
+  OrderUse use;
+  int rc = LOIKB_OK;
+  if (fused_queue && (rc = take_up_order(S, C, one_per_wave(F.kind), true, n_cur, &use, false))) return rc;
+  if (fused_queue)
+    hipLaunchKernelGGL(k_queue_init, grid1(std::max(std::max(C->ring_cap, n_cur), std::max(NCOUNTERS, ORDER_BINS))), dim3(256), 0, C->stream, C->d_ring, C->ring_cap,
+                       C->d_slots, n_cur, C->d_counters, NCOUNTERS, use.ordered ? (const int*)C->d_order : (const int*)nullptr, (unsigned int*)C->d_order_bins, ORDER_BINS);
+  else if (!queue_ready && small_flat) hipLaunchKernelGGL(k_queue_init, grid1(std::max(C->ring_cap, NCOUNTERS)), dim3(256), 0, C->stream, C->d_ring, C->ring_cap, C->d_slots, n_cur, C->d_counters, NCOUNTERS, (const int*)nullptr, (unsigned int*)nullptr, 0);
   else if (!queue_ready) HIPCHK(hipMemsetAsync(C->d_counters, 0, NCOUNTERS * sizeof(unsigned int), C->stream));
   if (!queue_ready) HIPCHK(hipEventRecord(C->ev_k0, C->stream));
-  OrderUse use;
-  int rc = take_up_order(S, C, !small_flat && whole_set && X.list == C->d_slots && n == n_cur && one_per_wave(F.kind), true, n_cur, &use);
-  if (rc) return rc;
+  if (!fused_queue && (rc = take_up_order(S, C, !small_flat && whole_set && X.list == C->d_slots && n == n_cur && one_per_wave(F.kind), true, n_cur, &use))) return rc;
   F.slice = flat_launch_slice(S, C, F.kind, F.mur, n, n_cur, use.ordered);
   F.nw = F.ndec;
   if (F.mur == 2) flat_table_window(S, F, n);
   if (F.mur == 0) { F.ndec = X.ndec; F.kexp_lo = X.kexp_lo; F.nw = F.ndec; F.dw0 = 0; }
-  const bool prep = F.kind == FlatKind::Flat2 && S->tune.flat_prep && F.ndec > 0 && F.mur != 1 && !S->opt.logging && whole_set && n == n_cur &&
-                    flat_prep_fits(S) && X.G == PREP_G && C->d_prep && (size_t)n_cur * flat_prep_stride(S->nc) * sizeof(double) <= C->d_prep.bytes();
+  const bool prep = flat_prep_route(S, C, n_cur) && F.ndec > 0 && whole_set && n == n_cur && X.G == PREP_G;
   if (prep) P.mode |= MODE_FLAT_PREP;
   F.prep = prep;
+  const bool decade0 = F.kexp_lo <= 0 && 0 < F.kexp_lo + F.ndec;
+  const bool virt = S->reset_pending != 0 && virtual_reset_route(S) && prep && (P.mode & MODE_ZERO_STATE) && !small_flat && X.cur == 0 && decade0;
+  F.virt = virt;
+  if (virt) S->reset_pending = 0;
+  else if ((rc = flush_pending_reset(S))) return rc;
   if (F.ndec > 0) {
     const dim3 hgrid((unsigned)((n + X.ipw - 1) / X.ipw));
     const size_t slds = (std::max((size_t)(WAVE + 1) * 22, (size_t)((F.small_na ? FLAT_NA_SMALL : FLAT_MAXA) + 1) * WAVE) + (size_t)(WAVE + 1) * 6 +
                          (size_t)X.ipw * S->nc * 21 + 16) * sizeof(T);
     auto* fslots = F.small_na ? k_fslots<T, FLAT_NA_SMALL> : k_fslots<T, FLAT_MAXA>;
-    hipLaunchKernelGGL(fslots, hgrid, dim3(WAVE), slds, C->stream, P, X.Bf, (const JointDesc*)S->d_jd, (const TailTopo*)S->d_topo,
+    Params<T> Pf = P;
+    if (virt) Pf.mode |= MODE_VIRTUAL_RESET;
+    hipLaunchKernelGGL(fslots, hgrid, dim3(WAVE), slds, C->stream, Pf, X.Bf, (const JointDesc*)S->d_jd, (const TailTopo*)S->d_topo,
                        (const int*)S->d_child_list, (const FlatLane*)S->flat.d_lanes, S->maxdepth, F.nanc, F.frows, S->flat.njmp, X.list, n,
                        X.G, C->d_fslots.as<T>(), F.kexp_lo, F.ndec, F.dw0, F.nw, F.mur == 2 ? C->d_fmask : (unsigned int*)nullptr,
                        prep ? C->d_prep.as<T>() : (T*)nullptr);
     HIPCHK(hipGetLastError());
   }
   if (!small_flat) HIPCHK(hipEventRecord(C->ev_k2, C->stream));
-  if (!small_flat) hipLaunchKernelGGL(k_ring_fill, grid1(C->ring_cap), dim3(256), 0, C->stream, C->d_ring, C->ring_cap, X.list, n, C->d_counters);
+  if (!small_flat && !fused_queue) hipLaunchKernelGGL(k_ring_fill, grid1(C->ring_cap), dim3(256), 0, C->stream, C->d_ring, C->ring_cap, X.list, n, C->d_counters);
   if ((rc = launch_flat_kernel(X, F))) return rc;
   P.mode = mode_keep;
   int* next = (X.list == C->d_slots) ? C->d_slots2 : C->d_slots;
   const bool small_finish = small_flat && S->tune.small_finish;
+  const bool order_pass = !small_flat && S->tune.flat_order && whole_set && n == n_cur && one_per_wave(F.kind) && !(S->opt.flags & LOIKB_OPT_FIXED_ITERS);
+  const bool fused_finish = fused_queue && order_pass;
   if (small_finish)
     hipLaunchKernelGGL(k_small_finish<T>, dim3(1), dim3(256), 0, C->stream, X.A.tiles, S->L, X.list, n, next, C->d_counters, NCOUNTERS, C->h_counters);
+  else if (fused_finish)
+    hipLaunchKernelGGL(k_finish_order<T>, grid1(n_cur), dim3(256), 0, C->stream, X.A.tiles, S->L, n_cur, S->opt.max_iter, next, C->d_counters + 3,
+                       (unsigned int*)C->d_order_bins, C->d_counters + ORDER_DEC_HIST);
   else
     hipLaunchKernelGGL(k_list_unfinished<T>, grid1(n), dim3(256), 0, C->stream, X.A.tiles, S->L, X.list, n, next, C->d_counters + 3);
   HIPCHK(hipGetLastError());
   C->stats.launches++; C->stats.tail_launches++; C->stats.lean_launches++; C->stats.flat_launches++;
   if (F.kind == FlatKind::Flat2) C->stats.flat_split_launches++;
   HIPCHK(hipEventRecord(C->ev_k1, C->stream));
-  const bool order_pass = !small_flat && S->tune.flat_order && whole_set && n == n_cur && one_per_wave(F.kind) && !(S->opt.flags & LOIKB_OPT_FIXED_ITERS);
   if (!order_pass && !small_finish) HIPCHK(hipMemcpyAsync(C->h_counters, C->d_counters, NCOUNTERS * sizeof(unsigned int), hipMemcpyDeviceToHost, C->stream));
-  if (order_pass && (rc = leave_order<T>(S, C, X.A, n_cur, true))) return rc;
+  if (order_pass && (rc = leave_order<T>(S, C, X.A, n_cur, true, fused_finish))) return rc;
   HIPCHK(hipStreamSynchronize(C->stream));
-  return flat_read_back(X, F, use, order_pass, small_finish, queue_ready, next);
+  return flat_read_back(X, F, use, order_pass, small_finish, queue_ready, next, fused_queue);
 }
 
 template <typename T>
@@ -2067,6 +2117,8 @@
   const int n = X.n, n_cur = X.n_cur, G = X.G, ipw = X.ipw, ndec = X.ndec, kexp_lo = X.kexp_lo;
   const int* list = X.list;
   const bool whole_set = X.whole_set, per_link = S->per_link;
+  int rc = flush_pending_reset(S);
+  if (rc) return rc;
   const size_t need = (size_t)n_cur * ndec * HSLOT_PAIRS * G * 2 * sizeof(T);
   if (need > C->d_hslots.bytes()) { g_last_error = "internal: decade-slot buffer smaller than the chunk"; return LOIKB_ERR_STATE; }
   const int waves_cu = S->plan.lean_waves_cu;
@@ -2081,8 +2133,7 @@
   const int wg_cap = wg_per_cu * std::max(1, (int)(S->ncu * ((double)C->B / (double)S->B) + 0.5));
   HIPCHK(hipEventRecord(C->ev_k0, C->stream));
   OrderUse use;
-  int rc = take_up_order(S, C, whole_set && list == C->d_slots && n == n_cur, whole_set, n_cur, &use);
-  if (rc) return rc;
+  if ((rc = take_up_order(S, C, whole_set && list == C->d_slots && n == n_cur, whole_set, n_cur, &use))) return rc;
   P.max_launch_iters = S->opt.max_iter + 1;
   const int wg_needed = (n + ipw * ltw - 1) / (ipw * ltw);
   const dim3 grid((unsigned)std::min(wg_needed, wg_cap));
@@ -2137,6 +2188,8 @@
   loikb_solver_impl* S = X.S; Chunk* C = X.C;
   const int n = X.n, n_cur = X.n_cur;
   const int cu_share = std::max(1, (int)(S->ncu * (TAIL_WAVES / tw) * ((double)C->B / (double)S->B) + 0.5));
+  int rc = flush_pending_reset(S);
+  if (rc) return rc;
   X.P.max_launch_iters = S->opt.max_iter + 1;
   const int wg_needed = (n + X.ipw * tw - 1) / (X.ipw * tw);
   const dim3 grid((unsigned)std::min(wg_needed, cu_share));
@@ -2144,8 +2197,7 @@
   HIPCHK(hipEventRecord(C->ev_k0, C->stream));
   const bool tail_whole = X.whole_set && X.list == C->d_slots && n == n_cur && !(S->opt.flags & LOIKB_OPT_FIXED_ITERS) && S->tune.flat_order;
   OrderUse use;
-  int rc = take_up_order(S, C, tail_whole, tail_whole, n_cur, &use);
-  if (rc) return rc;
+  if ((rc = take_up_order(S, C, tail_whole, tail_whole, n_cur, &use))) return rc;
   auto* kernel = S->href_diag ? k_tail<T, true> : k_tail<T, false>;
   hipLaunchKernelGGL(kernel, grid, dim3(WAVE * tw), lds, C->stream, X.P, X.Bf, (const JointDesc*)S->d_jd, (const TailTopo*)S->d_topo,
                      (const int*)S->d_child_list, S->maxdepth, S->maxchild, X.list, n, X.G);
@@ -2180,9 +2232,13 @@
   const bool flat_1pw = one_per_wave(flat_kind(S));
   const bool small_flat = whole_set && cur == 0 && S->chunks.size() == 1 && flat_1pw && flat_here && n_cur <= S->tune.flat_small_batch &&
                           n_cur >= std::max(1, S->tune.flat_min_batch);
-  if (whole_set && !small_flat) {
+  const bool flat_takes = flat_here && n_live >= (flat_1pw ? std::max(1, S->tune.flat_min_batch) : 64);
+  const bool list_pending = whole_set && !small_flat && S->tune.flat_seq && flat_takes && n_live == n_cur;
+  if (whole_set && !small_flat && !list_pending) {
     hipLaunchKernelGGL(k_list_iota, grid1(n_cur), dim3(256), 0, C->stream, C->d_slots, n_cur);
   } else if (!whole_set) {
+    int rc0 = flush_pending_reset(S);
+    if (rc0) return rc0;
     C->h_wave.resize(2 * (size_t)nw + 2);
     int* cnt = C->h_wave.data();
     int* off = cnt + nw + 1;
@@ -2197,6 +2253,7 @@
   HIPCHK(hipGetLastError());
   const int G = lanes_per_instance(S);
   TailCtx<T> X{S, C, P, make_bufs<T>(S, C, cur), A, cur, n_cur, whole_set, small_flat, G, WAVE / G, S->plan.ndec, S->plan.kexp_lo, C->d_slots, n_live};
+  X.list_pending = list_pending;
   P.B = n_cur;
   int tw = S->tune.tail_waves;
   while (tw > 1 && tw * tail_lds_bytes<T>(S->nc, G) > 160 * 1024) --tw;
@@ -2212,7 +2269,7 @@
   }
   int rc = LOIKB_OK;
   bool engine_ran = true;
-  if (flat_here && X.n >= (flat_1pw ? std::max(1, S->tune.flat_min_batch) : 64)) rc = launch_flat(X);
+  if (flat_takes) rc = launch_flat(X);
   else if (S->plan.lean && (P.mode & MODE_CACHE_H) && X.n >= 64) rc = launch_lean(X);
   else engine_ran = false;
   if (rc) return rc;
@@ -2278,6 +2335,9 @@
     C->stats.tail_instances = C->B;
     C->stats.tail_instance_iterations = tit;
     inst_iters = tit;
+  } else {
+    int rc = flush_pending_reset(S);
+    if (rc) return rc;
   }
   while (!direct_tail) {
     const int tiles_cur = (n_cur + WAVE - 1) / WAVE;
@@ -2469,7 +2529,7 @@
     return LOIKB_ERR_MU_STRATEGY;
   }
   int rc;
-  if (!S->plan.solve_ok && !bushy_goes_on_chip(S)) rc = run_pass_solve(S, false);
+  if (!S->plan.solve_ok && !bushy_goes_on_chip(S)) { if (!(rc = flush_pending_reset(S))) rc = run_pass_solve(S, false); }
   else if ((rc = start_mu(S))) {}
   else rc = S->f32 ? run_main_loop_t<float>(S) : run_main_loop_t<double>(S);
   return rc;
@@ -2836,6 +2896,13 @@
   if (!S->have_problem) { g_last_error = "Solve() before SolveInit()"; return LOIKB_ERR_STATE; }
   HIPCHK(hipSetDevice(S->device));
   int rc;
+  if (virtual_reset_route(S)) {
+    S->zero_state = true;
+    S->reset_pending = RS_RECURSION | RS_SOLVER;
+    rc = run_main_loop(S);
+    const int rc2 = flush_pending_reset(S);
+    return rc ? rc : rc2;
+  }
   if ((rc = reset_home(S, RS_RECURSION | RS_SOLVER, !S->opt.logging))) return rc;
   return S->opt.logging ? run_logged(S, RS_RECURSION | RS_SOLVER) : run_main_loop(S);
 }
@@ -3675,6 +3742,19 @@
   return LOIKB_OK;
 }
 
+int loikb_debug_flat_prep(loikb_solver* S, double* out, int n_inst, int* stride)
+{
+  if (!S || !out || !stride || n_inst < 0 || S->chunks.empty()) return LOIKB_ERR_ARG;
+  HIPCHK(hipSetDevice(S->device));
+  const Chunk& C = S->chunks[0];
+  *stride = flat_prep_stride(S->nc);
+  const size_t bytes = (size_t)n_inst * *stride * sizeof(double);
+  if (!C.d_prep || bytes > C.d_prep.bytes()) { g_last_error = "the handle has no prepared records of that many instances"; return LOIKB_ERR_STATE; }
+  HIPCHK(hipStreamSynchronize(S->stream));
+  HIPCHK(hipMemcpy(out, C.d_prep.as<double>(), bytes, hipMemcpyDeviceToHost));
+  return LOIKB_OK;
+}
+
 #ifdef LOIKB_TAIL_PROF
 int loikb_debug_wave_dbg(unsigned long long* out)
 {
diff --git a/loik_amd/csrc/loik_lean.hpp b/loik_amd/csrc/loik_lean.hpp
--- a/loik_amd/csrc/loik_lean.hpp
+++ b/loik_amd/csrc/loik_lean.hpp
@@ -827,11 +827,14 @@
 #endif
 
 #ifndef LOIKB_FLAT_KERNELS_TU
-__global__ void k_queue_init_iota(int* __restrict__ ring, int cap, int* __restrict__ list, int n, unsigned int* __restrict__ counters, int ncounters)
+__global__ void k_queue_init(int* __restrict__ ring, int cap, int* __restrict__ list, int n, unsigned int* __restrict__ counters, int ncounters,
+                             const int* __restrict__ order = nullptr, unsigned int* __restrict__ bins = nullptr, int nbins = 0)
 {
   const int i = blockIdx.x * blockDim.x + threadIdx.x;
-  if (i < cap) ring[i] = i < n ? i : -1;
-  if (i < n) list[i] = i;
+  const int slot = i < n ? (order != nullptr ? order[i] : i) : -1;
+  if (i < cap) ring[i] = slot;
+  if (i < n) list[i] = slot;
+  if (bins != nullptr && i < nbins) bins[i] = 0u;
   if (i < ncounters) {
     unsigned int v = 0u;
     if (i == LEAN_Q_TAIL) v = (unsigned int)n;
@@ -914,6 +917,29 @@
   __syncthreads();
   if (h[threadIdx.x]) atomicAdd(&bins[threadIdx.x], h[threadIdx.x]);
   if (dec_hist != nullptr && threadIdx.x < 32 && hd[threadIdx.x]) atomicAdd(&dec_hist[threadIdx.x], hd[threadIdx.x]);
+}
+template <typename T>
+__global__ void __launch_bounds__(256) k_finish_order(char* tiles, Layout L, int n, int max_iter, int* __restrict__ list_out,
+                                                      unsigned int* __restrict__ counter, unsigned int* __restrict__ bins,
+                                                      unsigned int* __restrict__ dec_hist)
+{
+  __shared__ unsigned int h[ORDER_BINS], hd[32];
+  h[threadIdx.x] = 0u;
+  if (threadIdx.x < 32) hd[threadIdx.x] = 0u;
+  __syncthreads();
+  const int b = blockIdx.x * blockDim.x + threadIdx.x;
+  if (b < n) {
+    const char* srec = lane_ptr<T>(tiles, L, b) + (size_t)L.off_s * pair_bytes<T>();
+    const int status = (int)ldp<T>(srec, SP_ST).x;
+    if (!(status & ST_DONE)) list_out[atomicAdd(counter, 1u)] = b;
+    if (!(status & (ST_CONVERGED | ST_PRIMAL_INF))) atomicAdd(counter + 1, 1u);
+    atomicAdd(&h[order_bin<T>(tiles, L, b, max_iter)], 1u);
+    const int kx = (int)ldp<T>(srec, SP_MU).y;
+    atomicAdd(&hd[kx < -16 ? 0 : kx > 15 ? 31 : kx + 16], 1u);
+  }
+  __syncthreads();
+  if (h[threadIdx.x]) atomicAdd(&bins[threadIdx.x], h[threadIdx.x]);
+  if (threadIdx.x < 32 && hd[threadIdx.x]) atomicAdd(&dec_hist[threadIdx.x], hd[threadIdx.x]);
 }
 #ifndef LOIKB_FLAT_KERNELS_TU
 __global__ void __launch_bounds__(ORDER_BINS) k_order_scan(unsigned int* __restrict__ bins)
```

Result: faster. 7.246 million (median of 6 runs) (+1.1%).
